# naimnv/cugraph-forked

Measured on AMD Instinct MI355X. Metric: PageRank edges/sec + BFS MTEPS on RMAT-24 at 1/2/4/8 MI355X, higher is better.
Workload: dtype f32

## Files before the change

cugraph-forked_amd/csrc/capi.hpp:

```cpp
#pragma once

#include "common.hpp"

#include <cugraph_c/algorithms.h>

#include <memory>
#include <string>
#include <cstring>
#include <vector>

namespace cgx {

struct mg_graph_t;
struct mg_context;

struct tuning_t {
  int pr_win_bits      = 0;
  bool pr_packed       = true;
  bool pr_whole        = true;
  bool pr_calib        = true;
  bool pr_deal_global  = false;
  bool pr_unit_w       = true;
  bool pr_fuse         = true;
  bool pr_enc          = true;
  bool pr_hub          = true;
  int64_t pr_band_cut  = -1;
  int pr_perm          = -1;
  int64_t pr_perm_cut  = -1;
  int pr_perm_span     = -1;
  int pr_share_div     = 0;
  bool pr_fast_build   = true;
  int mg_chunks        = 0;
  double bfs_alpha     = 40.0;
  double bfs_beta      = 64.0;
  double mg_bfs_alpha  = 40.0;
  double mg_bfs_beta   = 64.0;
  int mg_bfs_pipelined = 1;
  bool bfs_probe_vec   = true;
  bool bfs_head        = true;
  int bfs_res_grid     = 1024;
  int bfs_probe_grid   = 4096;
  int64_t bfs_td_cap   = 1024;
  bool louvain_hash    = true;
  bool louvain_big_hash = true;
  int louvain_big_cap  = 0;
  int64_t louvain_big_maxdeg = 0;
  bool louvain_wide_keys = false;
  double sssp_delta    = 0;
  int sssp_pull        = 0;
  int wcc_sample       = 2;
  int tc_path          = 0;
};

struct handle_t {
  int device         = 0;
  hipStream_t stream = nullptr;
  mg_context* mg     = nullptr;
  bool profiling     = false;
  tuning_t tune;
  size_t last_iterations     = 0;
  double last_hot_ms         = 0;
  size_t last_hot_launches   = 0;
  int64_t last_pr_stream     = 0;
  int64_t last_pr_permuted   = 0;
  size_t last_bfs_levels    = 0;
  size_t last_bfs_bottom_up  = 0;
  size_t last_louvain_levels = 0;
  double last_louvain_sweep_bytes = 0;
  int64_t last_louvain_local_edges = 0;
  int64_t last_louvain_ghosts      = 0;
  void* pinned = nullptr;
  std::vector<hipEvent_t> events;
  template <typename T>
  T* pinned_as()
  {
    static_assert(sizeof(T) <= kPinnedBytes, "pinned scratch too small");
    if (!pinned) HIP_CHECK(hipHostMalloc(&pinned, kPinnedBytes, hipHostMallocDefault));
    return static_cast<T*>(pinned);
  }
  void* polled = nullptr;
  template <typename T>
  T* polled_as()
  {
    static_assert(sizeof(T) <= kPinnedBytes, "polled scratch too small");
    if (!polled) {
      HIP_CHECK(hipHostMalloc(&polled, kPinnedBytes, hipHostMallocCoherent));
      std::memset(polled, 0, kPinnedBytes);
    }
    return static_cast<T*>(polled);
  }
  hipEvent_t event(size_t i)
  {
    while (events.size() <= i) {
      hipEvent_t e;
      HIP_CHECK(hipEventCreate(&e));
      events.push_back(e);
    }
    return events[i];
  }
  static constexpr size_t kPinnedBytes = 4096;
  ~handle_t()
  {
    if (pinned) (void)hipHostFree(pinned);
    if (polled) (void)hipHostFree(polled);
    for (auto e : events) (void)hipEventDestroy(e);
  }
};

struct array_view_t {
  void* data           = nullptr;
  size_t size          = 0;
  size_t num_bytes     = 0;
  data_type_id_t type  = INT32;
  template <typename T>
  T* as() const
  {
    return static_cast<T*>(data);
  }
};

struct device_array_t {
  buffer buf;
  size_t size         = 0;
  data_type_id_t type = INT32;
  device_array_t(size_t n, data_type_id_t t, hipStream_t s) : buf(n * dtype_size(t), s), size(n), type(t) {}
  array_view_t view() const { return array_view_t{buf.data(), size, size * dtype_size(type), type}; }
};

struct host_array_t {
  std::vector<std::byte> data;
  size_t size         = 0;
  data_type_id_t type = INT32;
};

struct err_t {
  std::string message;
};

struct pr_push_t {
  bool built = false;
  bool ok    = false;
  int win_bits = 12;
  buffer ent;
  buffer ew;
  bool packed = false;
  buffer ent16;
  buffer seg_base;
  buffer units;
  int64_t nunits = 0;
  buffer acc;
  int64_t nacc = 0;
  buffer items;
  buffer queue;
  std::vector<int64_t> qoff;
  int64_t nitems = 0;
  int64_t nwin   = 0;
  buffer tile_ctr;
  buffer win_multi;
  buffer win_items;
  buffer win_left;
  buffer empty_wins;
  int64_t nempty = 0, nwin_items = 0;
  buffer item_ticks;
  int calib = 0;
  bool bands = false;
  int64_t nwin_real = 0;
  buffer win_pub;
  buffer carry;
  buffer pos;
  int64_t perm_cut = 0;
  int64_t stream_len = 0;
  int last_iters = 0;
  double last_alpha = -1.0, last_eps = -1.0;
};

constexpr int64_t kIdxPad = 16;

struct adjacency_t {
  buffer offsets;
  buffer indices;
  buffer weights;
  bool idx_padded = false;
  bool degree_sorted = false;
  int64_t max_degree = -1;
  int unit_weights   = -1;
  bool sched_valid   = false;
  buffer order;
  std::vector<int64_t> bin_begin;
  buffer items;
  int64_t num_items = 0;
  buffer bfs_head;
  double wsum = -1;
  double sssp_delta = -1;
  int64_t sssp_eL = 0, sssp_eH = 0;
  buffer sssp_offL, sssp_offH, sssp_idxL, sssp_wL, sssp_idxH, sssp_wH, sssp_crowL, sssp_crowH;
  int64_t tc_edges = -1;
  buffer tc_ooff;
  buffer tc_oidx;
  pr_push_t pr;
};

struct graph_t {
  data_type_id_t vertex_type = INT32;
  data_type_id_t edge_type   = INT32;
  data_type_id_t weight_type = FLOAT32;
  bool store_transposed      = false;
  bool symmetric             = false;
  bool multigraph            = false;
  bool weighted              = false;
  bool renumbered            = false;
  bool multi_gpu             = false;
  int64_t num_vertices       = 0;
  int64_t num_edges          = 0;
  std::shared_ptr<adjacency_t> out;
  std::shared_ptr<adjacency_t> in;
  buffer number_map;
  bool ext_lookup_valid = false;
  buffer ext_sorted;
  buffer ext_internal;
  bool outw_valid = false;
  buffer outw;
  std::shared_ptr<mg_graph_t> mg;
};

struct centrality_result_t {
  std::unique_ptr<device_array_t> vertices;
  std::unique_ptr<device_array_t> values;
};

struct labeling_result_t {
  std::unique_ptr<device_array_t> vertices;
  std::unique_ptr<device_array_t> labels;
};

struct triangle_count_result_t {
  std::unique_ptr<device_array_t> vertices;
  std::unique_ptr<device_array_t> counts;
};

struct paths_result_t {
  std::unique_ptr<device_array_t> vertices;
  std::unique_ptr<device_array_t> distances;
  std::unique_ptr<device_array_t> predecessors;
};

struct extract_paths_result_t {
  size_t max_path_length = 0;
  std::unique_ptr<device_array_t> paths;
};

struct hits_result_t {
  std::unique_ptr<device_array_t> vertices;
  std::unique_ptr<device_array_t> hubs;
  std::unique_ptr<device_array_t> authorities;
  double hub_score_differences = 0;
  size_t number_of_iterations  = 0;
};

struct clustering_result_t {
  std::unique_ptr<device_array_t> vertices;
  std::unique_ptr<device_array_t> clusters;
  double modularity = 0;
  std::vector<std::unique_ptr<device_array_t>> levels;
};

inline handle_t* H(cugraph_resource_handle_t const* h) { return reinterpret_cast<handle_t*>(const_cast<cugraph_resource_handle_t*>(h)); }
inline graph_t* G(cugraph_graph_t* g) { return reinterpret_cast<graph_t*>(g); }
inline graph_t const* G(cugraph_graph_t const* g) { return reinterpret_cast<graph_t const*>(g); }
inline array_view_t const* AV(cugraph_type_erased_device_array_view_t const* v)
{
  return reinterpret_cast<array_view_t const*>(v);
}
inline array_view_t* AV(cugraph_type_erased_device_array_view_t* v) { return reinterpret_cast<array_view_t*>(v); }

inline cugraph_type_erased_device_array_view_t* new_view(device_array_t const* a)
{
  return reinterpret_cast<cugraph_type_erased_device_array_view_t*>(new array_view_t(a->view()));
}

template <typename F>
cugraph_error_code_t guarded(cugraph_error_t** error, F&& f)
{
  try {
    f();
    return CUGRAPH_SUCCESS;
  } catch (cgx::error const& e) {
    if (error) *error = reinterpret_cast<cugraph_error_t*>(new err_t{e.what()});
    return e.code;
  } catch (std::bad_alloc const& e) {
    if (error) *error = reinterpret_cast<cugraph_error_t*>(new err_t{std::string("allocation failed: ") + e.what()});
    return CUGRAPH_ALLOC_ERROR;
  } catch (std::exception const& e) {
    if (error) *error = reinterpret_cast<cugraph_error_t*>(new err_t{e.what()});
    return CUGRAPH_UNKNOWN_ERROR;
  }
}

void build_sg_graph(handle_t& h, graph_t& g, array_view_t const& src, array_view_t const& dst,
                    array_view_t const* weights, bool renumber);
adjacency_t& ensure_adjacency(handle_t& h, graph_t& g, bool transposed);
void ensure_schedule(handle_t& h, graph_t& g, adjacency_t& adj);
void renumber_ext_to_int(handle_t& h, graph_t& g, void* ids, size_t n, bool check);
void renumber_ext_to_int_unchecked(handle_t& h, graph_t& g, void* ids, size_t n);
void ensure_ext_lookup(handle_t& h, graph_t& g);
void unrenumber_int_to_ext(handle_t& h, graph_t& g, void* ids, size_t n);
std::unique_ptr<device_array_t> number_map_copy(handle_t& h, graph_t& g);
void const* out_weight_sums(handle_t& h, graph_t& g);

}
```

cugraph-forked_amd/csrc/capi_core.cpp:

```cpp
#include "capi.hpp"
#include "comm.hpp"

#include <cugraph_amd/ext.h>

#include <cstdlib>
#include <cstring>
#include <mutex>
#include <new>
#include <vector>

using namespace cgx;

namespace {

std::mutex g_stream_mutex;
std::vector<std::pair<int, hipStream_t>> g_free_streams;

void release_stream(int device, hipStream_t s)
{
  std::lock_guard<std::mutex> lk(g_stream_mutex);
  g_free_streams.emplace_back(device, s);
}

hipStream_t make_stream(int& device)
// ... 334 lines not shown
    CGX_EXPECTS(ps->type == INT32 || ps->type == INT64, CUGRAPH_UNSUPPORTED_TYPE_COMBINATION,
                "vertex type must be INT32 or INT64");
    auto g              = std::make_unique<graph_t>();
    g->vertex_type      = ps->type;
    g->edge_type        = ps->size < (size_t)INT32_MAX ? ps->type : INT64;
    g->weight_type      = pw ? pw->type : FLOAT32;
    g->weighted         = pw != nullptr;
    g->store_transposed = store_transposed == TRUE;
    g->symmetric        = properties ? properties->is_symmetric == TRUE : false;
    g->multigraph       = properties ? properties->is_multigraph == TRUE : false;
    build_sg_graph(*H(handle), *g, *ps, *pd, pw, renumber == TRUE);
    (void)check;
    *graph = reinterpret_cast<cugraph_graph_t*>(g.release());
  });
}

extern "C" void cugraph_sg_graph_free(cugraph_graph_t* graph)
{
  auto* g = G(graph);
  if (!g) return;
  (void)hipDeviceSynchronize();
  delete g;
}

extern "C" int64_t cugraph_amd_graph_get_number_of_vertices(const cugraph_graph_t* graph)
{
  return G(graph)->num_vertices;
}
extern "C" int64_t cugraph_amd_graph_get_number_of_edges(const cugraph_graph_t* graph) { return G(graph)->num_edges; }
extern "C" bool_t cugraph_amd_graph_is_symmetric(const cugraph_graph_t* graph)
{
  return G(graph)->symmetric ? TRUE : FALSE;
}

extern "C" cugraph_error_code_t cugraph_amd_device_array_views_copy(
  const cugraph_resource_handle_t* handle,
  size_t n,
  cugraph_type_erased_device_array_view_t* const* dst,
  const cugraph_type_erased_device_array_view_t* const* src,
  cugraph_error_t** error)
{
  *error = nullptr;
  return guarded(error, [&] {
    for (size_t i = 0; i < n; ++i) {
      auto* d       = AV(dst[i]);
      auto const* v = AV(src[i]);
      CGX_INPUT(d->type == v->type, "Invalid input argument: type mismatch");
      CGX_INPUT(d->size == v->size, "Invalid input argument: size mismatch");
    }
    for (size_t i = 0; i < n; ++i) {
      auto* d       = AV(dst[i]);
      auto const* v = AV(src[i]);
      if (v->num_bytes) HIP_CHECK(hipMemcpyAsync(d->data, v->data, v->num_bytes, hipMemcpyDefault, H(handle)->stream));
    }
    HIP_CHECK(hipStreamSynchronize(H(handle)->stream));
  });
}

extern "C" cugraph_error_code_t cugraph_amd_graph_get_adjacency(const cugraph_resource_handle_t* handle,
                                                               cugraph_graph_t* graph,
                                                               bool_t transposed,
                                                               cugraph_type_erased_device_array_t** offsets,
                                                               cugraph_type_erased_device_array_t** indices,
                                                               cugraph_type_erased_device_array_t** weights,
                                                               cugraph_error_t** error)
{
  *error = nullptr;
  return guarded(error, [&] {
    auto& h          = *H(handle);
    auto& g          = *G(graph);
    CGX_EXPECTS(!g.multi_gpu, CUGRAPH_NOT_IMPLEMENTED, "adjacency export is single-GPU only");
    adjacency_t& adj = ensure_adjacency(h, g, transposed == TRUE);
    size_t nv = (size_t)g.num_vertices, ne = (size_t)g.num_edges;
    auto o = new device_array_t(nv + 1, g.edge_type, h.stream);
    auto i = new device_array_t(ne, g.vertex_type, h.stream);
    HIP_CHECK(hipMemcpyAsync(o->buf.data(), adj.offsets.data(), (nv + 1) * dtype_size(g.edge_type),
                             hipMemcpyDeviceToDevice, h.stream));
    if (ne)
      HIP_CHECK(hipMemcpyAsync(i->buf.data(), adj.indices.data(), ne * dtype_size(g.vertex_type),
                               hipMemcpyDeviceToDevice, h.stream));
    *offsets = reinterpret_cast<cugraph_type_erased_device_array_t*>(o);
    *indices = reinterpret_cast<cugraph_type_erased_device_array_t*>(i);
    if (weights) {
      *weights = nullptr;
      if (g.weighted) {
        auto w = new device_array_t(ne, g.weight_type, h.stream);
        if (ne)
          HIP_CHECK(hipMemcpyAsync(w->buf.data(), adj.weights.data(), ne * dtype_size(g.weight_type),
                                   hipMemcpyDeviceToDevice, h.stream));
        *weights = reinterpret_cast<cugraph_type_erased_device_array_t*>(w);
      }
    }
    HIP_CHECK(hipStreamSynchronize(h.stream));
  });
}

extern "C" cugraph_error_code_t cugraph_amd_graph_get_out_weight_sums(const cugraph_resource_handle_t* handle,
                                                                     cugraph_graph_t* graph,
                                                                     cugraph_type_erased_device_array_t** sums,
                                                                     cugraph_error_t** error)
{
  *error = nullptr;
  *sums  = nullptr;
  return guarded(error, [&] {
    auto& h = *H(handle);
    auto& g = *G(graph);
    CGX_EXPECTS(!g.multi_gpu, CUGRAPH_NOT_IMPLEMENTED, "out-weight sums export is single-GPU only");
    size_t const nv = (size_t)g.num_vertices;
    void const* src = nv ? out_weight_sums(h, g) : nullptr;
    auto a          = new device_array_t(nv, g.weight_type, h.stream);
    if (nv)
      HIP_CHECK(hipMemcpyAsync(a->buf.data(), src, nv * dtype_size(g.weight_type), hipMemcpyDeviceToDevice, h.stream));
    HIP_CHECK(hipStreamSynchronize(h.stream));
    *sums = reinterpret_cast<cugraph_type_erased_device_array_t*>(a);
  });
}

extern "C" void cugraph_amd_set_profiling(cugraph_resource_handle_t* handle, bool_t enable)
{
  H(handle)->profiling = enable == TRUE;
}

extern "C" cugraph_error_code_t cugraph_amd_set_option(cugraph_resource_handle_t* handle, const char* name,
                                                       double value, cugraph_error_t** error)
{
  *error = nullptr;
  return guarded(error, [&] {
    CGX_INPUT(handle && name, "Invalid input argument: handle and name must not be NULL");
    tuning_t& t = H(handle)->tune;
    std::string const n(name);
    auto b   = [&](bool& f) { f = value != 0.0; };
    auto i32 = [&](int& f) { f = (int)value; };
    if (n == "pr_win_bits") {
      CGX_INPUT(value == 0 || value == 12 || value == 13 || value == 14 || value == 15,
                "Invalid input argument: pr_win_bits must be 0, 12, 13, 14 or 15");
      i32(t.pr_win_bits);
    } else if (n == "pr_packed") b(t.pr_packed);
    else if (n == "pr_whole") b(t.pr_whole);
    else if (n == "pr_calib") b(t.pr_calib);
    else if (n == "pr_deal_global") b(t.pr_deal_global);
    else if (n == "pr_unit_w") b(t.pr_unit_w);
    else if (n == "pr_fuse") b(t.pr_fuse);
    else if (n == "pr_enc") b(t.pr_enc);
    else if (n == "pr_hub") b(t.pr_hub);
    else if (n == "pr_band_cut") t.pr_band_cut = (int64_t)value;
    else if (n == "pr_perm") {
      CGX_INPUT(value == -1 || value == 0 || value == 1, "Invalid input argument: pr_perm must be -1, 0 or 1");
      i32(t.pr_perm);
    } else if (n == "pr_perm_cut") t.pr_perm_cut = (int64_t)value;
    else if (n == "pr_perm_span") {
      CGX_INPUT(value >= -1 && value <= 65536, "Invalid input argument: pr_perm_span must be in [-1, 65536]");
      i32(t.pr_perm_span);
    }
    else if (n == "pr_fast_build") b(t.pr_fast_build);
    else if (n == "pr_share_div") i32(t.pr_share_div);
    else if (n == "mg_chunks") i32(t.mg_chunks);
    else if (n == "sssp_pull") i32(t.sssp_pull);
    else if (n == "sssp_delta") {
      CGX_INPUT(value >= 0, "Invalid input argument: sssp_delta must be >= 0");
      t.sssp_delta = value;
    }
    else if (n == "wcc_sample") {
      CGX_INPUT(value >= 0 && value <= 64, "Invalid input argument: wcc_sample must be in [0, 64]");
      i32(t.wcc_sample);
    }
    else if (n == "tc_path") {
      CGX_INPUT(value == 0 || value == 1 || value == 2, "Invalid input argument: tc_path must be 0, 1 or 2");
      i32(t.tc_path);
    }
    else if (n == "bfs_alpha") t.bfs_alpha = value;
    else if (n == "bfs_beta") t.bfs_beta = value;
    else if (n == "mg_bfs_alpha") t.mg_bfs_alpha = value;
    else if (n == "mg_bfs_beta") t.mg_bfs_beta = value;
    else if (n == "mg_bfs_pipelined") i32(t.mg_bfs_pipelined);
    else if (n == "bfs_probe_vec") b(t.bfs_probe_vec);
    else if (n == "bfs_head") b(t.bfs_head);
    else if (n == "bfs_res_grid") i32(t.bfs_res_grid);
    else if (n == "bfs_probe_grid") i32(t.bfs_probe_grid);
    else if (n == "bfs_td_cap") t.bfs_td_cap = (int64_t)value;
    else if (n == "louvain_hash") b(t.louvain_hash);
    else if (n == "louvain_big_hash") b(t.louvain_big_hash);
    else if (n == "louvain_big_cap") i32(t.louvain_big_cap);
    else if (n == "louvain_big_maxdeg") t.louvain_big_maxdeg = (int64_t)value;
    else if (n == "louvain_wide_keys") b(t.louvain_wide_keys);
    else if (n == "defaults") t = tuning_t{};
    else fail(CUGRAPH_INVALID_INPUT, "Invalid input argument: unknown option " + n);
  });
}
extern "C" size_t cugraph_amd_last_iterations(const cugraph_resource_handle_t* handle)
{
  return H(handle)->last_iterations;
}
extern "C" double cugraph_amd_last_hot_kernel_ms(const cugraph_resource_handle_t* handle)
{
  return H(handle)->last_hot_ms;
}
extern "C" size_t cugraph_amd_last_hot_kernel_launches(const cugraph_resource_handle_t* handle)
{
  return H(handle)->last_hot_launches;
}
extern "C" void cugraph_amd_last_pagerank_schedule(const cugraph_resource_handle_t* handle, int64_t* stream_entries,
                                                   int64_t* permuted_vertices)
{
  *stream_entries    = H(handle)->last_pr_stream;
  *permuted_vertices = H(handle)->last_pr_permuted;
}
extern "C" size_t cugraph_amd_last_bfs_levels(const cugraph_resource_handle_t* handle)
{
  return H(handle)->last_bfs_levels;
}
extern "C" size_t cugraph_amd_last_bfs_bottom_up_steps(const cugraph_resource_handle_t* handle)
{
  return H(handle)->last_bfs_bottom_up;
}
extern "C" size_t cugraph_amd_last_louvain_levels(const cugraph_resource_handle_t* handle)
{
  return H(handle)->last_louvain_levels;
}
extern "C" double cugraph_amd_last_louvain_sweep_bytes(const cugraph_resource_handle_t* handle)
{
  return H(handle)->last_louvain_sweep_bytes;
}
extern "C" void cugraph_amd_last_louvain_partition(const cugraph_resource_handle_t* handle, int64_t* local_edges,
                                                   int64_t* ghosts)
{
  *local_edges = H(handle)->last_louvain_local_edges;
  *ghosts      = H(handle)->last_louvain_ghosts;
}
extern "C" size_t cugraph_amd_trim_device_cache(void) { return cgx::device_cache_trim(); }
extern "C" void cugraph_amd_allocator_stats(double* out) { cgx::device_alloc_stats(out); }
extern "C" const char* cugraph_amd_version(void) { return "cugraph-forked_amd libcugraph_c gfx950 " __DATE__; }
```

cugraph-forked_amd/csrc/pagerank.hip:

```cpp
#include "capi.hpp"
#include "comm.hpp"
#include "mg_graph.hpp"
#include "prims.hpp"
#include "schedule.hpp"

#include <rocprim/device/device_reduce_by_key.hpp>
#include <rocprim/iterator/counting_iterator.hpp>
#include <rocprim/iterator/transform_iterator.hpp>

#include <algorithm>
#include <cmath>
#include <cstdlib>

#if defined(__HIP_DEVICE_COMPILE__) && !defined(__GFX9__)
#error "s_waitcnt vmcnt(0) orders stores on gfx9-family (gfx950) targets only"
#endif

namespace cgx {

struct pr_state {
  double base;
  double pers_factor;
  double diff;
  double prev_diff;
// ... 236 lines not shown
      s1 += (double)x1 * (double)a.wgt[e + w];
    } else {
      s0 += (double)x0;
      s1 += (double)x1;
    }
  }
  if (e < end) {
    R x0 = a.x_in[a.idx[e]];
    if constexpr (WEIGHTED) s0 += (double)x0 * (double)a.wgt[e];
    else s0 += (double)x0;
  }
  return s0 + s1;
}

template <typename V, typename E, typename R, bool WEIGHTED>
__device__ __forceinline__ double row_partial_block(pr_args<V, E, R> const& a, E beg, E end, int tid)
{
  double s0 = 0, s1 = 0, s2 = 0, s3 = 0;
  E e = beg + tid;
  for (; e + 3 * 256 < end; e += 4 * 256) {
    V u0 = a.idx[e], u1 = a.idx[e + 256], u2 = a.idx[e + 512], u3 = a.idx[e + 768];
    R x0 = a.x_in[u0], x1 = a.x_in[u1], x2 = a.x_in[u2], x3 = a.x_in[u3];
    if constexpr (WEIGHTED) {
      s0 += (double)x0 * (double)a.wgt[e];
      s1 += (double)x1 * (double)a.wgt[e + 256];
      s2 += (double)x2 * (double)a.wgt[e + 512];
      s3 += (double)x3 * (double)a.wgt[e + 768];
    } else {
      s0 += (double)x0;
      s1 += (double)x1;
      s2 += (double)x2;
      s3 += (double)x3;
    }
  }
  for (; e < end; e += 256) {
    R x0 = a.x_in[a.idx[e]];
    if constexpr (WEIGHTED) s0 += (double)x0 * (double)a.wgt[e];
    else s0 += (double)x0;
  }
  return (s0 + s1) + (s2 + s3);
}

template <typename V, typename E, typename R, typename Acc = unsigned long long>
__device__ __forceinline__ void vertex_update_from(pr_args<V, E, R> const& a, V v, double s, R old, R ow, double base,
                                                   double pf, Acc& my_diff, Acc& my_dang)
{
  double n = base + a.alpha * s;
  if (a.pers) n += pf * (double)a.pers[v];
  R nr     = (R)n;
  a.pr[v]  = nr;
  acc_add(my_diff, fabs((double)nr - (double)old));
  R xv = R(0);
  if (ow == R(0)) acc_add(my_dang, (double)nr);
  else xv = (R)((double)nr / (double)ow);
  store_x<R>(a.x_out, x_index(a, (int64_t)v), xv, a.enc);
}

template <typename V, typename E, typename R, typename Acc = unsigned long long>
__device__ __forceinline__ void vertex_update(pr_args<V, E, R> const& a, V v, double s, double base, double pf,
                                              Acc& my_diff, Acc& my_dang)
{
  vertex_update_from<V, E, R, Acc>(a, v, s, a.pr[v], a.outw[v], base, pf, my_diff, my_dang);
}

template <typename V, typename E, typename R, bool WEIGHTED>
__global__ __launch_bounds__(256) void k_pr_iter(pr_args<V, E, R> a)
{
  __shared__ double sm[4];
  if (a.st->done) return;
  work_item const it = a.items[blockIdx.x];
  double const base  = a.st->base;
  double const pf    = a.st->pers_factor;
  double my_diff = 0, my_dang = 0;
  int const tid = threadIdx.x;
  if (it.width == 256) {
    for (int64_t p = it.begin; p < it.end; ++p) {
      V v      = a.order ? a.order[p] : (V)p;
      double s = row_partial_block<V, E, R, WEIGHTED>(a, a.off[v], a.off[v + 1], tid);
      s        = block_sum_256(s, sm);
      if (tid == 0) vertex_update<V, E, R, double>(a, v, s, base, pf, my_diff, my_dang);
    }
  } else {
    int const w      = it.width;
    int const lane   = tid & (w - 1);
    int const group  = tid / w;
    int const groups = 256 / w;
    for (int64_t p0 = it.begin; p0 < it.end; p0 += groups) {
      int64_t p  = p0 + group;
      bool valid = p < it.end;
      double s   = 0;
      V v        = 0;
      if (valid) {
        v = a.order ? a.order[p] : (V)p;
        s = row_partial<V, E, R, WEIGHTED>(a, a.off[v], a.off[v + 1], lane, w);
      }
      for (int o = w >> 1; o > 0; o >>= 1) s += __shfl_xor(s, o, 64);
      if (valid && lane == 0) vertex_update<V, E, R, double>(a, v, s, base, pf, my_diff, my_dang);
    }
  }
  finish_iteration<V, E, R>(a, my_diff, my_dang, true);
}

constexpr int kPushThreads = 1024;
constexpr int kPerThread   = 8;
constexpr int kPushUnit    = kPerThread * kPushThreads;
constexpr int kQueues      = 8;
constexpr int kTileUnits   = 8;
constexpr int kGroupItems  = 128;
constexpr int kCtrStride   = 32;
constexpr int kPushBlocks  = 512;
constexpr int kCommCUs     = 16;
constexpr int kHubBytes = 32768 - 512;
#ifndef CGX_APPLY_BATCH
#define CGX_APPLY_BATCH 4
#endif
template <typename R>
__host__ __device__ constexpr double fix_scale()
{
  return sizeof(R) == 8 ? 4611686018427387904.0  : 4503599627370496.0 ;
}
template <typename R>
__host__ __device__ constexpr double fix_scale_inv()
{
  return 1.0 / fix_scale<R>();
}

inline int push_win_bits(int64_t n_rows, tuning_t const& tu, bool wide = false)
{
  if (tu.pr_win_bits == 12 || tu.pr_win_bits == 13 || tu.pr_win_bits == 14) return tu.pr_win_bits;
  if (tu.pr_win_bits == 15) return wide ? 15 : 14;
  if (n_rows >= (int64_t(1) << 24)) return wide ? 15 : 14;
  return n_rows >= (int64_t(1) << 23) ? 14 : n_rows >= (int64_t(1) << 22) ? 13 : 12;
}

inline int64_t push_band_cut(int64_t n, tuning_t const& tu)
{
  if (tu.pr_band_cut >= 0) return tu.pr_band_cut;
  (void)n;
  return 0;
}

inline bool push_perm_on(int win_bits, tuning_t const& tu)
{
  if (tu.pr_perm >= 0) return tu.pr_perm != 0;
  return win_bits == 14;
}
inline int push_perm_span(int win_bits, tuning_t const& tu)
{
  (void)win_bits;
  return tu.pr_perm_span >= 0 ? tu.pr_perm_span : 1;
}
constexpr int64_t kPermCut = int64_t(1) << 20;

inline int push_blocks(int win_bits) { return win_bits >= 14 ? kPushBlocks / 2 : kPushBlocks; }

constexpr int64_t kShareDiv = 4;

struct push_unit {
  int64_t k0, k1;
  int64_t base;
  int64_t win;
};

template <typename V, typename E, typename R>
struct push_args {
  pr_args<V, E, R> a;
  uint32_t const* ent;
  R const* ew;
  uint16_t const* ent16;
  uint32_t const* seg_base;
  push_unit const* units;
  int64_t nunits;
  unsigned long long* acc;
  uint32_t* carry;
  int64_t const* items;
  int64_t const* queue;
  int64_t qoff[kQueues + 1];
  int64_t nitems;
  unsigned int* tile_ctr;
  uint8_t const* win_multi;
  int keep_acc;
  int win_bits;
  int64_t nwin;
  int fuse;
  int parity;
  uint32_t* win_left;
  uint32_t const* win_items;
  int64_t const* empty_wins;
  int64_t nempty;
  int64_t nwin_items;
  int bands;
  int64_t nwin_real;
  uint32_t* win_pub;
  int64_t nhub;
  unsigned long long* tl;
  int64_t tl_cap;
  int launch;
  uint32_t* item_ticks;
};

template <typename T>
__device__ __forceinline__ T nt_load(T const* p)
{
  return __builtin_nontemporal_load(p);
}

template <typename R>
__device__ __forceinline__ unsigned long long to_fixed(double v)
{
  return (unsigned long long)__double2ll_rn(v * fix_scale<R>());
}

__device__ __forceinline__ unsigned long long to_fixed_f32(float x)
{
  float const y     = x * 1048576.0f;
  uint32_t const hi = (uint32_t)y;
  float const fr    = y - (float)hi;
  uint32_t const lo = (uint32_t)__builtin_rintf(fr * 4294967296.0f);
  return ((unsigned long long)hi << 32) | lo;
}

template <typename R>
__device__ __forceinline__ unsigned long long fixed_of(R x)
{
  if constexpr (std::is_same<R, float>::value) return to_fixed_f32(x);
  else return to_fixed<R>((double)x);
}

constexpr int64_t kWholeItem = int64_t(1) << 40;
constexpr int64_t kWinMask   = kWholeItem - 1;

template <int WB, typename V, typename E, typename R, typename A>
__device__ __forceinline__ void flush_window(push_args<V, E, R> const& sa, A* acc, int64_t win_w)
{
  __syncthreads();
  unsigned long long* g = sa.acc + ((win_w & kWinMask) << WB);
  if (win_w & kWholeItem) {
    for (int i = threadIdx.x; i < (1 << WB); i += kPushThreads) {
      g[i]   = (unsigned long long)acc[i];
      acc[i] = 0;
    }
  } else {
    for (int i = threadIdx.x; i < (1 << WB); i += kPushThreads) {
      unsigned long long v = (unsigned long long)acc[i];
      if (v) {
        atomicAdd(g + i, v);
        acc[i] = 0;
      }
    }
  }
  __syncthreads();
}

__device__ __forceinline__ void wait_vmem() { asm volatile("s_waitcnt vmcnt(0)" ::: "memory"); }

template <int WB, typename V, typename E, typename R, typename A>
__device__ __forceinline__ void apply_window(push_args<V, E, R> const& sa, int64_t w, A* lds,
                                             unsigned long long& my_diff, unsigned long long& my_dang)
{
  auto const& a     = sa.a;
  double const base = a.st->base;
  double const pf   = a.st->pers_factor;
  int64_t const v0  = w << WB;
  int const n       = (int)min((int64_t)1 << WB, a.nv - v0);
  constexpr int kB = WB >= 14 ? 4 : 1;
  for (int i0 = threadIdx.x; i0 < n; i0 += kB * kPushThreads) {
    unsigned long long f[kB];
    R old[kB], ow[kB];
#pragma unroll
    for (int j = 0; j < kB; ++j) {
      int const i = i0 + j * kPushThreads;
      if (i < n) {
        if (lds) {
          f[j]   = (unsigned long long)lds[i];
          lds[i] = 0;
        } else {
          f[j] = __hip_atomic_exchange(sa.acc + v0 + i, 0ull, __ATOMIC_RELAXED, __HIP_MEMORY_SCOPE_AGENT);
        }
        if constexpr (WB == 15)
          f[j] += (unsigned long long)__hip_atomic_exchange(sa.carry + v0 + i, 0u, __ATOMIC_RELAXED,
                                                            __HIP_MEMORY_SCOPE_AGENT) << 32;
        old[j] = a.pr[v0 + i];
        ow[j]  = a.outw[v0 + i];
      }
    }
#pragma unroll
    for (int j = 0; j < kB; ++j) {
      int const i = i0 + j * kPushThreads;
      if (i < n)
        vertex_update_from<V, E, R>(a, (V)(v0 + i), (double)(long long)f[j] * fix_scale_inv<R>(), old[j], ow[j], base, pf,
                                    my_diff, my_dang);
    }
  }
}

template <int WB, typename V, typename E, typename R>
__device__ __forceinline__ void apply_window_banded(push_args<V, E, R> const& sa, int64_t rw, unsigned long long* lds,
                                                    int64_t own_vw, unsigned long long& my_diff,
                                                    unsigned long long& my_dang)
{
  auto const& a     = sa.a;
  double const base = a.st->base;
  double const pf   = a.st->pers_factor;
  int64_t const v0  = rw << WB;
  int const n       = (int)min((int64_t)1 << WB, a.nv - v0);
  int64_t const vw0 = rw, vw1 = rw + sa.nwin_real;
  bool const multi0 = sa.win_multi[vw0] != 0, multi1 = sa.win_multi[vw1] != 0;
  unsigned long long* const p0 = sa.acc + (vw0 << WB);
  unsigned long long* const p1 = sa.acc + (vw1 << WB);
  auto plane = [&](unsigned long long* p, bool multi, int i) -> unsigned long long {
    return multi ? __hip_atomic_exchange(p + i, 0ull, __ATOMIC_RELAXED, __HIP_MEMORY_SCOPE_AGENT)
                 : __hip_atomic_load(p + i, __ATOMIC_RELAXED, __HIP_MEMORY_SCOPE_AGENT);
  };
  constexpr int kB = 2;
  for (int i0 = threadIdx.x; i0 < n; i0 += kB * kPushThreads) {
    unsigned long long f[kB];
    R old[kB], ow[kB];
#pragma unroll
    for (int j = 0; j < kB; ++j) {
      int const i = i0 + j * kPushThreads;
      if (i < n) {
        unsigned long long x0, x1;
        if (lds && own_vw == vw0) {
// ... 147 lines not shown
    fused_finish<WB, V, E, R, true>(sa, acc, win_w);
    return;
  }
  if constexpr (FUSE) {
    if (sa.fuse) {
      fused_finish<WB, V, E, R>(sa, acc, win_w);
      return;
    }
  }
  flush_window<WB, V, E, R>(sa, acc, win_w);
}

template <int WB, typename V, typename E, typename R, bool WEIGHTED>
__device__ __forceinline__ void push_body(push_args<V, E, R> const& sa)
{
  constexpr int kWin = 1 << WB;
  __shared__ unsigned long long acc[kWin];
  __shared__ int64_t s_item;
  __shared__ unsigned long long s_t0;
  if (sa.a.st->done) return;
  int const tid = threadIdx.x;
  for (int i = tid; i < kWin; i += kPushThreads) acc[i] = 0ull;
  using cunit_t        = __attribute__((address_space(4))) push_unit const;
  cunit_t* const units = (cunit_t*)sa.units;
  R const* const x     = sa.a.x_in;
  int q                = (int)(blockIdx.x % kQueues);
  for (int tries = 0; tries < kQueues;) {
    if (tid == 0) {
      if (sa.item_ticks) s_t0 = __builtin_amdgcn_s_memrealtime();
      int64_t const i = (int64_t)atomicAdd(sa.tile_ctr + (sa.parity * kQueues + q) * kCtrStride, 1u);
      s_item          = i < sa.qoff[q + 1] - sa.qoff[q] ? sa.queue[sa.qoff[q] + i] : -1;
    }
    __syncthreads();
    int64_t const it = s_item;
    __syncthreads();
    if (it < 0) {
      q = (q + 1) % kQueues;
      ++tries;
      continue;
    }
    int64_t const ua = sa.items[it], ub = sa.items[it + 1];
    int64_t const win = units[ua].win;
    int64_t k0   = units[ua].k0;
    int n        = (int)(units[ua].k1 - k0);
    int64_t base = units[ua].base;
    uint32_t ent[kPerThread];
    R w[kPerThread];
#pragma unroll
    for (int j = 0; j < kPerThread; ++j) {
      ent[j] = nt_load(sa.ent + k0 + j * kPushThreads + tid);
      if constexpr (WEIGHTED) w[j] = nt_load(sa.ew + k0 + j * kPushThreads + tid);
    }
    for (int64_t un = ua; un < ub; ++un) {
      R const* const xb = x + base;
      R xv[kPerThread];
#pragma unroll
      for (int j = 0; j < kPerThread; ++j) {
        bool const ok = j * kPushThreads + tid < n;
        xv[j]         = xb[ok ? (ent[j] >> WB) : 0u];
        xv[j]         = ok ? xv[j] : R(0);
      }
      int64_t const nx  = un + 1 < ub ? un + 1 : un;
      int64_t const k0n = units[nx].k0;
      int const nn      = (int)(units[nx].k1 - k0n);
      int64_t const bsn = units[nx].base;
      uint32_t ent_n[kPerThread];
      R w_n[kPerThread];
#pragma unroll
      for (int j = 0; j < kPerThread; ++j) {
        ent_n[j] = nt_load(sa.ent + k0n + j * kPushThreads + tid);
        if constexpr (WEIGHTED) w_n[j] = nt_load(sa.ew + k0n + j * kPushThreads + tid);
      }
      __builtin_amdgcn_sched_barrier(0);
#pragma unroll
      for (int j = 0; j < kPerThread; ++j) {
        if constexpr (WEIGHTED) {
          atomicAdd(&acc[ent[j] & (kWin - 1)], to_fixed<R>((double)xv[j] * (double)w[j]));
        } else {
          atomicAdd(&acc[ent[j] & (kWin - 1)], fixed_of(xv[j]));
        }
      }
#pragma unroll
      for (int j = 0; j < kPerThread; ++j) {
        ent[j] = ent_n[j];
        if constexpr (WEIGHTED) w[j] = w_n[j];
      }
      n    = nn;
      base = bsn;
    }
    end_item<WB, V, E, R, (WB >= 14)>(sa, acc, win);
    if (sa.item_ticks && tid == 0) sa.item_ticks[s_item] = (uint32_t)(__builtin_amdgcn_s_memrealtime() - s_t0);
  }
}

template <int WB, typename V, typename E, typename R, bool WEIGHTED>
__global__ __launch_bounds__(kPushThreads, 8) void k_pr_push_q(push_args<V, E, R> sa)
{
  push_body<WB, V, E, R, WEIGHTED>(sa);
}

template <int WB, typename V, typename E, typename R, bool WEIGHTED>
__global__ __launch_bounds__(kPushThreads) void k_pr_push_q_wide(push_args<V, E, R> sa)
{
  push_body<WB, V, E, R, WEIGHTED>(sa);
}

constexpr int kSegEntries = 512;
typedef unsigned int u32x4_t __attribute__((ext_vector_type(4)));

__host__ __device__ __forceinline__ int64_t seg_store_index(int64_t p)
{
  int64_t const e = p & (kSegEntries - 1);
  return (p & ~(int64_t)(kSegEntries - 1)) | ((e & 63) << 3) | (e >> 6);
}
constexpr int kSegsPerUnit = kPushUnit / kSegEntries;

__device__ __forceinline__ uint32_t wave_incl_scan(uint32_t v)
{
  v += (uint32_t)__builtin_amdgcn_update_dpp(0, (int)v, 0x111, 0xf, 0xf, false);
  v += (uint32_t)__builtin_amdgcn_update_dpp(0, (int)v, 0x112, 0xf, 0xf, false);
  v += (uint32_t)__builtin_amdgcn_update_dpp(0, (int)v, 0x114, 0xf, 0xf, false);
  v += (uint32_t)__builtin_amdgcn_update_dpp(0, (int)v, 0x118, 0xf, 0xf, false);
  v += (uint32_t)__builtin_amdgcn_update_dpp(0, (int)v, 0x142, 0xa, 0xf, false);
  v += (uint32_t)__builtin_amdgcn_update_dpp(0, (int)v, 0x143, 0xc, 0xf, false);
  return v;
}

template <int N>
__device__ __forceinline__ void wave_incl_scan_rows(uint32_t (&v)[N])
{
#pragma unroll
  for (int j = 0; j < N; ++j) v[j] += (uint32_t)__builtin_amdgcn_update_dpp(0, (int)v[j], 0x111, 0xf, 0xf, false);
#pragma unroll
  for (int j = 0; j < N; ++j) v[j] += (uint32_t)__builtin_amdgcn_update_dpp(0, (int)v[j], 0x112, 0xf, 0xf, false);
#pragma unroll
  for (int j = 0; j < N; ++j) v[j] += (uint32_t)__builtin_amdgcn_update_dpp(0, (int)v[j], 0x114, 0xf, 0xf, false);
#pragma unroll
  for (int j = 0; j < N; ++j) v[j] += (uint32_t)__builtin_amdgcn_update_dpp(0, (int)v[j], 0x118, 0xf, 0xf, false);
#pragma unroll
  for (int j = 0; j < N; ++j) v[j] += (uint32_t)__builtin_amdgcn_update_dpp(0, (int)v[j], 0x142, 0xa, 0xf, false);
#pragma unroll
  for (int j = 0; j < N; ++j) v[j] += (uint32_t)__builtin_amdgcn_update_dpp(0, (int)v[j], 0x143, 0xc, 0xf, false);
}

template <int WB, typename V, typename E, typename R, bool ENC, bool HUB = false, bool FUSE = false, bool BANDS = false>
__device__ __forceinline__ void push_body16(push_args<V, E, R> const& sa)
{
  using xw_t = typename std::conditional<ENC, uint32_t, R>::type;
  constexpr int kWin        = 1 << WB;
  constexpr uint32_t kJump  = (1u << (16 - WB)) - 1;
  constexpr uint32_t kLow   = (1u << WB) - 1;
  constexpr int kRows       = kSegEntries / 64;
  static_assert(kRows == kPerThread, "a wave segment is one unit row per thread");
  constexpr bool kAcc32 = WB == 15;
  using acc_t           = typename std::conditional<kAcc32, uint32_t, unsigned long long>::type;
  __shared__ acc_t acc[kWin];
  constexpr int kHub = HUB ? kHubBytes / (int)sizeof(xw_t) : 1;
  __shared__ xw_t hub[kHub];
  __shared__ int64_t s_item;
  __shared__ unsigned long long s_t0;
  if (sa.a.st->done) return;
  int const tid  = threadIdx.x;
  int const lane = tid & 63;
  int const wave = __builtin_amdgcn_readfirstlane(tid >> 6);
  for (int i = tid; i < kWin; i += kPushThreads) acc[i] = 0;
  using cunit_t        = __attribute__((address_space(4))) push_unit const;
  cunit_t* const units = (cunit_t*)sa.units;
  xw_t const* const x  = reinterpret_cast<xw_t const*>(sa.a.x_in);
  uint32_t const nh    = HUB ? (uint32_t)min((int64_t)kHub, sa.nhub) : 0u;
  if constexpr (HUB)
    for (uint32_t i = tid; i < nh; i += kPushThreads) hub[i] = x[i];
  int q                = (int)(blockIdx.x % kQueues);
  for (int tries = 0; tries < kQueues;) {
    if (tid == 0) {
      if (sa.tl || sa.item_ticks) s_t0 = __builtin_amdgcn_s_memrealtime();
      int64_t const i = (int64_t)atomicAdd(sa.tile_ctr + (sa.parity * kQueues + q) * kCtrStride, 1u);
      s_item          = i < sa.qoff[q + 1] - sa.qoff[q] ? sa.queue[sa.qoff[q] + i] : -1;
    }
    __syncthreads();
    int64_t const it = s_item;
    __syncthreads();
    if (it < 0) {
      q = (q + 1) % kQueues;
      ++tries;
      continue;
    }
    int64_t const ua = sa.items[it], ub = sa.items[it + 1];
    int64_t const win = units[ua].win;
    auto seg_ptr = [&](int64_t u) {
      return reinterpret_cast<u32x4_t const*>(sa.ent16 + units[u].k0 + wave * kSegEntries) + lane;
    };
    auto seg_n = [&](int64_t u) { return (int)(units[u].k1 - units[u].k0) - wave * kSegEntries; };
    auto entry = [&](u32x4_t const& w, int j) { return (w[j >> 1] >> ((j & 1) * 16)) & 0xFFFFu; };
    auto gather = [&](u32x4_t const& w, uint32_t base, xw_t (&xv)[kRows]) {
      uint32_t sc[kRows];
#pragma unroll
      for (int j = 0; j < kRows; ++j) {
        uint32_t const e = entry(w, j);
        sc[j]            = (e >> WB) == kJump ? (e & kLow) : (e >> WB);
      }
      wave_incl_scan_rows<kRows>(sc);
      uint32_t run = base;
      if constexpr (HUB) {
        uint32_t src[kRows];
#pragma unroll
        for (int j = 0; j < kRows; ++j) {
          src[j] = run + sc[j];
          run += (uint32_t)__builtin_amdgcn_readlane((int)sc[j], 63);
        }
        if (run < nh) {
#pragma unroll
          for (int j = 0; j < kRows; ++j) xv[j] = hub[src[j]];
        } else {
#pragma unroll
          for (int j = 0; j < kRows; ++j) xv[j] = x[src[j]];
        }
        return;
      }
#pragma unroll
      for (int j = 0; j < kRows; ++j) {
        uint32_t const src = run + sc[j];
        run += (uint32_t)__builtin_amdgcn_readlane((int)sc[j], 63);
        xv[j] = x[src];
      }
    };
    auto sum = [&](u32x4_t const& w, xw_t const (&xv)[kRows]) {
      if constexpr (kAcc32) {
        uint32_t lo[kRows], old[kRows];
        uint32_t* const cw = sa.carry + ((win & kWinMask) << WB);
#pragma unroll
        for (int j = 0; j < kRows; ++j) {
          uint32_t const e = entry(w, j);
          unsigned long long fix;
          if constexpr (ENC) fix = dec_fixed(xv[j]);
          else fix = fixed_of(xv[j]);
          lo[j] = (e >> WB) != kJump ? (uint32_t)fix : 0u;
          if ((e >> WB) != kJump) {
            old[j] = atomicAdd(&acc[e & kLow], lo[j]);
            if (fix >> 32) atomicAdd(cw + (e & kLow), (uint32_t)(fix >> 32));
          }
        }
#pragma unroll
        for (int j = 0; j < kRows; ++j) {
          uint32_t const e = entry(w, j);
          if ((e >> WB) != kJump && old[j] > ~lo[j]) atomicAdd(cw + (e & kLow), 1u);
        }
      } else {
#pragma unroll
        for (int j = 0; j < kRows; ++j) {
          uint32_t const e = entry(w, j);
          xw_t const v     = xv[j];
          unsigned long long fix;
          if constexpr (ENC) fix = dec_fixed(v);
          else fix = fixed_of(v);
          if ((e >> WB) != kJump) atomicAdd(&acc[e & kLow], fix);
        }
      }
    };
    int64_t const u1 = ua + 1 < ub ? ua + 1 : ua;
    int nA      = seg_n(ua);
    int nB      = seg_n(u1);
    uint32_t bB = __builtin_amdgcn_readfirstlane(sa.seg_base[u1 * kSegsPerUnit + wave]);
    u32x4_t wA  = nt_load(seg_ptr(ua));
    u32x4_t wB  = nt_load(seg_ptr(u1));
    xw_t xA[kRows];
    if (nA > 0) gather(wA, __builtin_amdgcn_readfirstlane(sa.seg_base[ua * kSegsPerUnit + wave]), xA);
    for (int64_t un = ua; un < ub; ++un) {
      bool const actB = un + 1 < ub && nB > 0;
      xw_t xB[kRows];
      if (actB) gather(wB, bB, xB);
      int64_t const u2  = un + 2 < ub ? un + 2 : un;
      int const n2      = seg_n(u2);
      uint32_t const b2 = sa.seg_base[u2 * kSegsPerUnit + wave];
      u32x4_t const e2  = nt_load(seg_ptr(u2));
      __builtin_amdgcn_sched_barrier(0);
      if (nA > 0) sum(wA, xA);
      wA = wB;
#pragma unroll
      for (int j = 0; j < kRows; ++j) xA[j] = xB[j];
      nA = actB ? nB : 0;
      wB = e2;
      nB = n2;
      bB = __builtin_amdgcn_readfirstlane(b2);
    }
    end_item<WB, V, E, R, FUSE, BANDS>(sa, acc, win);
    if (sa.item_ticks && tid == 0) sa.item_ticks[s_item] = (uint32_t)(__builtin_amdgcn_s_memrealtime() - s_t0);
    if (sa.tl && tid == 0) {
      unsigned long long const t_end = __builtin_amdgcn_s_memrealtime();
      unsigned long long const k     = atomicAdd(sa.tl, 1ull);
      if ((int64_t)k < sa.tl_cap) {
        unsigned long long* r = sa.tl + 1 + 4 * k;
        r[0] = ((unsigned long long)sa.launch << 32) | blockIdx.x;
        int64_t const iu = s_item;
        r[1] = ((unsigned long long)(units[sa.items[iu + 1] - 1].k1 - units[sa.items[iu]].k0) << 32) | (unsigned long long)iu;
        r[2] = s_t0;
        r[3] = t_end;
      }
    }
  }
}

template <int WB, typename V, typename E, typename R, bool ENC>
__global__ __launch_bounds__(kPushThreads, 8) void k_pr_push16(push_args<V, E, R> sa)
{
  push_body16<WB, V, E, R, ENC>(sa);
}

template <typename V, typename E, typename R, bool ENC, bool BANDS = false>
__global__ __launch_bounds__(kPushThreads) void k_pr_push16_w14(push_args<V, E, R> sa)
{
  push_body16<14, V, E, R, ENC, true, true, BANDS>(sa);
}

template <typename V, typename E, typename R, bool ENC>
__global__ __launch_bounds__(kPushThreads) void k_pr_push16_w15(push_args<V, E, R> sa)
{
  push_body16<15, V, E, R, ENC, true, true, false>(sa);
}

template <typename V, typename E, typename R, bool WEIGHTED>
__global__ __launch_bounds__(kPushThreads) void k_pr_push_q_w14(push_args<V, E, R> sa)
{
  push_body<14, V, E, R, WEIGHTED>(sa);
}

template <typename V, typename E, typename R>
__global__ __launch_bounds__(256) void k_pr_apply(push_args<V, E, R> sa)
{
  auto const& a = sa.a;
  if (sa.tile_ctr && blockIdx.x == 0 && threadIdx.x < kQueues)
    sa.tile_ctr[(sa.parity * kQueues + threadIdx.x) * kCtrStride] = 0u;
  if (a.st->done) return;
  double const base = a.st->base;
  double const pf   = a.st->pers_factor;
  unsigned long long my_diff = 0, my_dang = 0;
  int64_t const stride = (int64_t)gridDim.x * blockDim.x;
  int64_t v            = blockIdx.x * (int64_t)blockDim.x + threadIdx.x;
  auto take_carry = [&](int64_t vv) -> unsigned long long {
    if (!sa.carry) return 0ull;
    uint32_t const c = sa.carry[vv];
    if (c) sa.carry[vv] = 0u;
    return (unsigned long long)c << 32;
  };
  if constexpr (std::is_same<R, float>::value) {
    typedef float f4_t __attribute__((ext_vector_type(4)));
    typedef unsigned u4_t __attribute__((ext_vector_type(4)));
    typedef unsigned long long u2_t __attribute__((ext_vector_type(2)));
    bool const aligned = ((reinterpret_cast<uintptr_t>(a.pr) | reinterpret_cast<uintptr_t>(a.outw) |
                           reinterpret_cast<uintptr_t>(a.x_out) | reinterpret_cast<uintptr_t>(sa.acc)) & 15) == 0 &&
                         !sa.carry;
    if (aligned) {
      int64_t const nq = a.nv / 4;
      for (int64_t q = v; q < nq; q += stride) {
        u2_t const f01 = reinterpret_cast<u2_t const*>(sa.acc)[2 * q];
        u2_t const f23 = reinterpret_cast<u2_t const*>(sa.acc)[2 * q + 1];
        f4_t const old = reinterpret_cast<f4_t const*>(a.pr)[q];
        f4_t const ow  = reinterpret_cast<f4_t const*>(a.outw)[q];
        unsigned long long const f[4] = {f01.x, f01.y, f23.x, f23.y};
        float const o[4] = {old.x, old.y, old.z, old.w}, w[4] = {ow.x, ow.y, ow.z, ow.w};
        float nr[4], xv[4];
#pragma unroll
        for (int j = 0; j < 4; ++j) {
          int64_t const vj = 4 * q + j;
          double n = base + a.alpha * ((double)(long long)f[j] * fix_scale_inv<R>());
          if (a.pers) n += pf * (double)a.pers[vj];
          nr[j] = (float)n;
          acc_add(my_diff, fabs((double)nr[j] - (double)o[j]));
          xv[j] = 0.0f;
          if (w[j] == 0.0f) acc_add(my_dang, (double)nr[j]);
          else xv[j] = (float)((double)nr[j] / (double)w[j]);
          if (!sa.keep_acc && f[j] && (!sa.win_multi || sa.win_multi[vj >> sa.win_bits])) sa.acc[vj] = 0ull;
        }
        reinterpret_cast<f4_t*>(a.pr)[q] = f4_t{nr[0], nr[1], nr[2], nr[3]};
        if (a.pos) {
          u4_t const p = reinterpret_cast<u4_t const*>(a.pos)[q];
          uint32_t const v4 = (uint32_t)(4 * q);
          if (p.x != v4 || p.y != v4 + 1 || p.z != v4 + 2 || p.w != v4 + 3) {
            store_x<R>(a.x_out, p.x, xv[0], a.enc);
            store_x<R>(a.x_out, p.y, xv[1], a.enc);
            store_x<R>(a.x_out, p.z, xv[2], a.enc);
            store_x<R>(a.x_out, p.w, xv[3], a.enc);
            continue;
          }
        }
        if (a.enc)
          reinterpret_cast<u4_t*>(a.x_out)[q] = u4_t{enc_fixed(xv[0]), enc_fixed(xv[1]), enc_fixed(xv[2]), enc_fixed(xv[3])};
        else
          reinterpret_cast<f4_t*>(a.x_out)[q] = f4_t{xv[0], xv[1], xv[2], xv[3]};
      }
      v = 4 * nq + blockIdx.x * (int64_t)blockDim.x + threadIdx.x;
    }
  }
  constexpr int kApplyBatch = CGX_APPLY_BATCH;
  for (; v + (kApplyBatch - 1) * stride < a.nv; v += kApplyBatch * stride) {
    unsigned long long f[kApplyBatch];
    R old[kApplyBatch], ow[kApplyBatch];
#pragma unroll
    for (int j = 0; j < kApplyBatch; ++j) {
      f[j]   = sa.acc[v + j * stride];
      old[j] = a.pr[v + j * stride];
      ow[j]  = a.outw[v + j * stride];
    }
#pragma unroll
    for (int j = 0; j < kApplyBatch; ++j) {
      int64_t const vj = v + j * stride;
      if (!sa.keep_acc && f[j] && (!sa.win_multi || sa.win_multi[vj >> sa.win_bits])) sa.acc[vj] = 0ull;
      f[j] += take_carry(vj);
      vertex_update_from<V, E, R>(a, (V)vj, (double)(long long)f[j] * fix_scale_inv<R>(), old[j], ow[j], base, pf, my_diff,
                                  my_dang);
    }
  }
  for (; v < a.nv; v += stride) {
    unsigned long long f = sa.acc[v];
    if (!sa.keep_acc && f && (!sa.win_multi || sa.win_multi[v >> sa.win_bits])) sa.acc[v] = 0ull;
    f += take_carry(v);
    vertex_update<V, E, R>(a, (V)v, (double)(long long)f * fix_scale_inv<R>(), base, pf, my_diff, my_dang);
  }
  finish_iteration<V, E, R>(a, my_diff, my_dang, true);
}

constexpr int kRowsTile = 4096;
template <typename E>
__device__ __forceinline__ int64_t row_of_edge(E const* off, int64_t lo, int64_t hi, int64_t e)
{
  while (lo < hi) {
    int64_t const mid = (lo + hi + 1) >> 1;
    if ((int64_t)off[mid] <= e) lo = mid;
    else hi = mid - 1;
  }
  return lo;
}

template <typename E>
__global__ __launch_bounds__(256) void k_edge_rows(E const* off, int64_t nv, int64_t ne, uint32_t* rows)
{
  __shared__ int64_t s_r[2];
  __shared__ E s_off[kRowsTile + 1];
  for (int64_t e0 = (int64_t)blockIdx.x * kRowsTile; e0 < ne; e0 += (int64_t)gridDim.x * kRowsTile) {
    int64_t const e1 = min(e0 + kRowsTile, ne);
    if (threadIdx.x == 0) {
      s_r[0] = row_of_edge(off, 0, nv - 1, e0);
      s_r[1] = row_of_edge(off, s_r[0], nv - 1, e1 - 1);
    }
    __syncthreads();
    int64_t const r0 = s_r[0], r1 = s_r[1];
    bool const staged = r1 - r0 < kRowsTile;
    if (staged)
// ... 146 lines not shown
  }
}

template <typename KC = key_w32>
__global__ void k_jump_counts(uint64_t const* keys, int64_t ne, int64_t const* ws, uint32_t dmax, uint32_t pmax,
                              uint32_t* mj, KC kc = {})
{
  for (int64_t k = blockIdx.x * (int64_t)blockDim.x + threadIdx.x; k < ne; k += (int64_t)gridDim.x * blockDim.x) {
    int64_t const w     = kc.win(keys[k]);
    uint32_t const prev = k == ws[w] ? 0u : kc.src(keys[k - 1]);
    uint32_t const D    = kc.src(keys[k]) - prev;
    mj[k]               = D > dmax ? (D + pmax - 1) / pmax : 0u;
  }
}

struct jump_count_p {
  uint64_t const* keys;
  int64_t const* ws;
  int64_t ne;
  key_p kc;
  uint32_t dmax, pmax;
  __device__ __forceinline__ uint32_t operator()(int64_t k) const
  {
    if (k >= ne) return 0u;
    uint64_t const key  = keys[k];
    int64_t const w     = kc.win(key);
    uint32_t const prev = k == ws[w] ? 0u : kc.src(keys[k - 1]);
    uint32_t const D    = kc.src(key) - prev;
    return D > dmax ? (D + pmax - 1) / pmax : 0u;
  }
};

__global__ void k_pack16(uint64_t const* keys, uint32_t const* vals, uint32_t const* rows, int64_t ne,
                         int64_t const* ws, uint32_t const* mj, unsigned long long const* cm,
                         unsigned long long const* pb, int wb, uint32_t pmax,
                         uint16_t* ent16)
{
  uint32_t const jump = (1u << (16 - wb)) - 1, low = (1u << wb) - 1;
  for (int64_t k = blockIdx.x * (int64_t)blockDim.x + threadIdx.x; k < ne; k += (int64_t)gridDim.x * blockDim.x) {
    int64_t const w     = (int64_t)(keys[k] >> 32);
    uint32_t const prev = k == ws[w] ? 0u : (uint32_t)keys[k - 1];
    uint32_t const D    = (uint32_t)keys[k] - prev;
    uint32_t const m    = mj[k];
    int64_t const pos   = k + (int64_t)cm[k] + (int64_t)pb[w];
    uint32_t const slot = rows[vals[k]] & low;
    if (m == 0) {
      ent16[seg_store_index(pos)] = (uint16_t)((D << wb) | slot);
    } else {
      for (uint32_t j = 0; j < m; ++j) {
        uint32_t const pay                  = j + 1 < m ? pmax : D - pmax * (m - 1);
        ent16[seg_store_index(pos - m + j)] = (uint16_t)((jump << wb) | pay);
      }
      ent16[seg_store_index(pos)] = (uint16_t)slot;
    }
  }
}

template <typename CM>
__global__ void k_pack16_p(uint64_t const* keys, int64_t ne, int64_t const* ws, CM const* cm,
                           unsigned long long const* pb, key_p kc, uint32_t pmax, uint16_t* ent16)
{
  int const wb        = kc.wb;
  uint32_t const jump = (1u << (16 - wb)) - 1;
  for (int64_t k = blockIdx.x * (int64_t)blockDim.x + threadIdx.x; k < ne; k += (int64_t)gridDim.x * blockDim.x) {
    uint64_t const key  = keys[k];
    int64_t const w     = kc.win(key);
    uint32_t const prev = k == ws[w] ? 0u : kc.src(keys[k - 1]);
    uint32_t const D    = kc.src(key) - prev;
    uint32_t const m    = (uint32_t)(cm[k] - cm[k - 1]);
    int64_t const pos   = k + (int64_t)cm[k] + (int64_t)pb[w];
    uint32_t const slot = kc.slot(key);
    if (m == 0) {
      ent16[seg_store_index(pos)] = (uint16_t)((D << wb) | slot);
    } else {
      for (uint32_t j = 0; j < m; ++j) {
        uint32_t const pay                  = j + 1 < m ? pmax : D - pmax * (m - 1);
        ent16[seg_store_index(pos - m + j)] = (uint16_t)((jump << wb) | pay);
      }
      ent16[seg_store_index(pos)] = (uint16_t)slot;
    }
  }
}

template <typename CM>
__device__ __forceinline__ int64_t packed_start(int64_t const* ws, CM const* cm, int64_t w, int64_t nwin, int64_t total)
{
  return w == nwin ? total : ws[w] + (ws[w] > 0 ? (int64_t)cm[ws[w] - 1] : 0);
}
template <typename CM>
__global__ void k_packed_pads(int64_t const* ws, CM const* cm, int64_t nwin, int64_t total, unsigned long long* pad)
{
  for (int64_t w = blockIdx.x * (int64_t)blockDim.x + threadIdx.x; w <= nwin; w += (int64_t)gridDim.x * blockDim.x) {
    int64_t const len = w == nwin ? 0 : packed_start(ws, cm, w + 1, nwin, total) - packed_start(ws, cm, w, nwin, total);
    pad[w]            = (unsigned long long)((kSegEntries - len % kSegEntries) % kSegEntries);
  }
}
template <typename CM>
__global__ void k_packed_win_starts(int64_t const* ws, CM const* cm, unsigned long long const* pb, int64_t nwin,
                                    int64_t total, int64_t* nws)
{
  for (int64_t w = blockIdx.x * (int64_t)blockDim.x + threadIdx.x; w <= nwin; w += (int64_t)gridDim.x * blockDim.x)
    nws[w] = packed_start(ws, cm, w, nwin, total) + (int64_t)pb[w];
}

__global__ void k_unit_counts(int64_t const* nws, int64_t nwin, uint32_t* cnt)
{
  for (int64_t w = blockIdx.x * (int64_t)blockDim.x + threadIdx.x; w <= nwin; w += (int64_t)gridDim.x * blockDim.x)
    cnt[w] = w == nwin ? 0u : (uint32_t)((nws[w + 1] - nws[w] + kPushUnit - 1) / kPushUnit);
}
__global__ void k_units_direct(int64_t const* nws, int64_t nwin, uint32_t const* upos, int64_t nunits,
                               push_unit* units)
{
  for (int64_t u = blockIdx.x * (int64_t)blockDim.x + threadIdx.x; u < nunits; u += (int64_t)gridDim.x * blockDim.x) {
    int64_t lo = 0, hi = nwin - 1;
    while (lo < hi) {
      int64_t const mid = (lo + hi + 1) >> 1;
      if ((int64_t)upos[mid] <= u) lo = mid;
      else hi = mid - 1;
    }
    units[u] = push_unit{nws[lo] + (u - (int64_t)upos[lo]) * kPushUnit, 0, 0, lo};
  }
}

__global__ void k_packed_unit_marks(int64_t const* nws, int64_t nwin, uint32_t* flag)
{
  for (int64_t w = blockIdx.x * (int64_t)blockDim.x + threadIdx.x; w < nwin; w += (int64_t)gridDim.x * blockDim.x)
    for (int64_t p = nws[w]; p < nws[w + 1]; p += kPushUnit) flag[p] = 1u;
}
__global__ void k_packed_unit_heads(uint32_t const* flag, uint32_t const* uid, int64_t total, int64_t const* nws,
                                    int64_t nwin, push_unit* units)
{
  for (int64_t p = blockIdx.x * (int64_t)blockDim.x + threadIdx.x; p < total; p += (int64_t)gridDim.x * blockDim.x) {
    if (!flag[p]) continue;
    int64_t lo = 0, hi = nwin - 1;
    while (lo < hi) {
      int64_t mid = (lo + hi + 1) >> 1;
      if (nws[mid] <= p) lo = mid;
      else hi = mid - 1;
    }
    units[uid[p]] = push_unit{p, 0, 0, lo};
  }
}

template <typename KC, typename CM>
__global__ void k_seg_bases(push_unit const* units, int64_t nunits, uint64_t const* keys, int64_t ne,
                            int64_t const* ws, uint32_t const* mj, CM const* cm, unsigned long long const* pb,
                            uint32_t dmax, uint32_t pmax, uint32_t* seg_base, KC kc)
{
  int64_t const n = nunits * kSegsPerUnit;
  for (int64_t i = blockIdx.x * (int64_t)blockDim.x + threadIdx.x; i < n; i += (int64_t)gridDim.x * blockDim.x) {
    push_unit const u = units[i / kSegsPerUnit];
    int64_t const p   = u.k0 + (i % kSegsPerUnit) * kSegEntries;
    uint32_t base     = 0;
    if (p < u.k1) {
      int64_t lo = 0, hi = ne - 1;
      while (lo < hi) {
        int64_t mid = (lo + hi) >> 1;
        if (mid + (int64_t)cm[mid] + (int64_t)pb[kc.win(keys[mid])] < p) lo = mid + 1;
        else hi = mid;
      }
      int64_t const k     = lo;
      uint32_t const m    = mj ? mj[k] : (uint32_t)(cm[k] - cm[k - 1]);
      int64_t const w     = kc.win(keys[k]);
      int64_t const j     = p - (k + (int64_t)cm[k] + (int64_t)pb[w] - m);
      uint32_t const prev = k == ws[w] ? 0u : kc.src(keys[k - 1]);
      uint32_t const src  = kc.src(keys[k]);
      uint32_t const D    = src - prev;
      base = j < (int64_t)m ? prev + pmax * (uint32_t)j : src - (m ? 0u : (D <= dmax ? D : 0u));
    }
    seg_base[i] = base;
  }
}

inline void mark_whole_items(hipStream_t s, pr_push_t& pp, push_unit* units, std::vector<push_unit>& hu,
                             std::vector<int64_t> const& item_u, int64_t nitems, tuning_t const& tu)
{
  int64_t const nunits = (int64_t)hu.size();
  bool const no_whole  = !tu.pr_whole;
  std::vector<uint8_t> multi((size_t)std::max<int64_t>(pp.nwin, 1), 0);
  for (int64_t i = 0; i < nitems; ++i) {
    int64_t const u = item_u[i], last = item_u[i + 1] - 1;
    int64_t const wu = hu[u].win & kWinMask;
    bool const whole = !no_whole && (u == 0 || (hu[u - 1].win & kWinMask) != wu) &&
                       (last + 1 >= nunits || (hu[last + 1].win & kWinMask) != wu);
    CGX_EXPECTS(!(hu[u].win & kWholeItem), CUGRAPH_UNKNOWN_ERROR, "mark_whole_items: unit already flagged");
    if (whole) hu[u].win |= kWholeItem;
    else multi[wu] = 1;
  }
  to_device(units, hu.data(), (size_t)nunits, s);
  {
    int64_t const nreal = pp.bands ? pp.nwin_real : pp.nwin;
    std::vector<uint32_t> cnt((size_t)std::max<int64_t>(nreal, 1), 0u);
    for (int64_t i = 0; i < nitems; ++i) {
      int64_t const wu = hu[item_u[i]].win & kWinMask;
      if (wu < pp.nwin) ++cnt[pp.bands ? wu % nreal : wu];
    }
    std::vector<int64_t> empty;
    pp.nwin_items = 0;
    for (int64_t w = 0; w < nreal; ++w) {
      if (cnt[w]) ++pp.nwin_items;
      else empty.push_back(w);
    }
    if (pp.bands) {
      pp.win_pub.set_stream(s);
      pp.win_pub.resize(cnt.size() * sizeof(uint32_t));
      HIP_CHECK(hipMemsetAsync(pp.win_pub.data(), 0, cnt.size() * sizeof(uint32_t), s));
    }
    pp.nempty = (int64_t)empty.size();
    pp.win_items.set_stream(s);
    pp.win_items.resize(cnt.size() * sizeof(uint32_t));
    to_device(pp.win_items.data<uint32_t>(), cnt.data(), cnt.size(), s);
    pp.win_left.set_stream(s);
    pp.win_left.resize(cnt.size() * sizeof(uint32_t));
    pp.empty_wins.set_stream(s);
    pp.empty_wins.resize(std::max<size_t>(empty.size(), 1) * sizeof(int64_t));
    if (!empty.empty()) to_device(pp.empty_wins.data<int64_t>(), empty.data(), empty.size(), s);
    HIP_CHECK(hipStreamSynchronize(s));
  }
  pp.win_multi.set_stream(s);
  pp.win_multi.resize(multi.size());
  to_device(pp.win_multi.data<uint8_t>(), multi.data(), multi.size(), s);
  HIP_CHECK(hipStreamSynchronize(s));
}

inline void upload_items(hipStream_t s, pr_push_t& pp, std::vector<int64_t> const& item_u,
                         std::vector<int64_t> const& queue, int64_t nitems)
{
  pp.items.set_stream(s);
  pp.items.resize(item_u.size() * sizeof(int64_t));
  to_device(pp.items.data<int64_t>(), item_u.data(), item_u.size(), s);
  pp.queue.set_stream(s);
  pp.queue.resize(std::max<size_t>(queue.size(), 1) * sizeof(int64_t));
  to_device(pp.queue.data<int64_t>(), queue.data(), queue.size(), s);
  pp.nitems = nitems;
}

inline void build_items(hipStream_t s, pr_push_t& pp, push_unit* units, int64_t nunits, bool xcd_queues,
                        tuning_t const& tu)
{
  int64_t const ne = nunits ? to_host(&units[nunits - 1].k1, 1, s)[0] : 0;
  auto hu = to_host(units, nunits, s);
  int64_t const div = tu.pr_share_div > 0 ? tu.pr_share_div : kShareDiv;
  int64_t const tg  = std::max<int64_t>(kPushUnit, ne / (push_blocks(pp.win_bits) * div));
  std::vector<int64_t> item_u, item_e;
  for (int64_t u0 = 0; u0 < nunits;) {
    int64_t u1 = u0;
    while (u1 < nunits && hu[u1].win == hu[u0].win) ++u1;
    int64_t const size = hu[u1 - 1].k1 - hu[u0].k0;
    int64_t const n    = std::max<int64_t>(1, (size + tg / 2) / tg);
    int64_t k          = 0;
    for (int64_t u = u0; u < u1; ++u) {
      int64_t const done = hu[u].k0 - hu[u0].k0;
      bool const head    = u == u0 || (xcd_queues ? (k < n && done * n >= k * size) : (u - u0) % kTileUnits == 0);
      if (head) {
        item_u.push_back(u);
        item_e.push_back(0);
        ++k;
      }
      item_e.back() += hu[u].k1 - hu[u].k0;
    }
    u0 = u1;
  }
  int64_t const nitems = (int64_t)item_u.size();
  item_u.push_back(nunits);
  std::vector<int64_t> queue;
  queue.reserve(nitems);
  if (xcd_queues) {
    int64_t const ngroups = (nitems + kGroupItems - 1) / kGroupItems;
    std::vector<int64_t> gsize(ngroups, 0), gorder(ngroups);
    for (int64_t i = 0; i < nitems; ++i) gsize[i / kGroupItems] += item_e[i];
    for (int64_t g = 0; g < ngroups; ++g) gorder[g] = g;
    std::stable_sort(gorder.begin(), gorder.end(), [&](int64_t a, int64_t b) { return gsize[a] > gsize[b]; });
    std::vector<int> gq(ngroups, 0);
    int64_t load[kQueues] = {};
    for (int64_t g : gorder) {
      int best = 0;
      for (int q = 1; q < kQueues; ++q)
        if (load[q] < load[best]) best = q;
      gq[g] = best;
      load[best] += gsize[g];
    }
    for (int q = 0; q < kQueues; ++q) {
      pp.qoff[q] = (int64_t)queue.size();
      for (int64_t i = 0; i < nitems; ++i)
        if (gq[i / kGroupItems] == q) queue.push_back(i);
    }
  } else {
    for (int64_t i = 0; i < nitems; ++i) queue.push_back(i);
    pp.qoff[0] = 0;
    for (int q = 1; q < kQueues; ++q) pp.qoff[q] = nitems;
  }
  pp.qoff[kQueues] = (int64_t)queue.size();
  mark_whole_items(s, pp, units, hu, item_u, nitems, tu);
  upload_items(s, pp, item_u, queue, nitems);
}

constexpr int kCalGroup = 16;

inline bool calibration_wanted(pr_push_t const& pp, tuning_t const& tu)
{
  return pp.calib == 0 && pp.nitems > 0 && tu.pr_calib;
}

inline void calibrate_queues(hipStream_t s, pr_push_t& pp, tuning_t const& tu)
{
  int64_t const n = pp.nitems;
  auto t          = to_host(pp.item_ticks.data<uint32_t>(), n, s);
  std::vector<int64_t> queue;
  queue.reserve(n);
  if (tu.pr_deal_global || pp.win_bits < 13) {
    for (int64_t i = 0; i < n; ++i) queue.push_back(i);
    std::stable_sort(queue.begin(), queue.end(), [&](int64_t a, int64_t b) { return t[a] > t[b]; });
    pp.qoff.assign(kQueues + 1, n);
    pp.qoff[0] = 0;
  } else {
    int64_t const G  = kCalGroup;
    int64_t const ng = (n + G - 1) / G;
    std::vector<uint64_t> gc(ng, 0);
    for (int64_t i = 0; i < n; ++i) gc[i / G] += t[i];
    std::vector<int64_t> go(ng);
    for (int64_t g = 0; g < ng; ++g) go[g] = g;
    std::stable_sort(go.begin(), go.end(), [&](int64_t a, int64_t b) { return gc[a] > gc[b]; });
    std::vector<std::vector<int64_t>> qg(kQueues);
    uint64_t load[kQueues] = {};
    for (int64_t g : go) {
      int best = 0;
      for (int q = 1; q < kQueues; ++q)
        if (load[q] < load[best]) best = q;
      qg[best].push_back(g);
      load[best] += gc[g];
    }
    if (pp.bands) {
      std::vector<int> gband(ng, 0);
      {
        auto hu = to_host(pp.units.data<push_unit>(), (size_t)pp.nunits, s);
        auto iu = to_host(pp.items.data<int64_t>(), (size_t)n, s);
        for (int64_t g = 0; g < ng; ++g) gband[g] = (hu[iu[g * G]].win & kWinMask) >= pp.nwin_real ? 1 : 0;
      }
      for (auto& l : qg) std::stable_sort(l.begin(), l.end(), [&](int64_t a, int64_t b) { return gband[a] < gband[b]; });
    }
    pp.qoff.assign(kQueues + 1, 0);
    for (int q = 0; q < kQueues; ++q) {
      pp.qoff[q] = (int64_t)queue.size();
      for (int64_t g : qg[q])
        for (int64_t i = g * G; i < std::min(n, (g + 1) * G); ++i) queue.push_back(i);
    }
    pp.qoff[kQueues] = n;
  }
  to_device(pp.queue.data<int64_t>(), queue.data(), queue.size(), s);
  HIP_CHECK(hipStreamSynchronize(s));
  pp.calib = 2;
}

template <typename C, typename R>
void build_push_from_coo(hipStream_t s, uint32_t const* rows, C const* cols, R const* w, int64_t ne, int64_t n_rows,
                         int64_t n_cols, pr_push_t& pp, tuning_t const& tu, bool col_sorted = false,
                         int64_t band_cut = 0, bool wide = false)
{
  pp.built = true;
  pp.ok    = (uint64_t)n_rows < (1ull << 32) && (uint64_t)n_cols < (1ull << 32) && (uint64_t)ne < (1ull << 32);
  if (!pp.ok) return;
  int const wb = push_win_bits(n_rows, tu, wide && !w && tu.pr_packed);
  int const sb = 32 - wb;
  if (wb != 14 || w || !tu.pr_packed || band_cut >= n_cols) band_cut = 0;
  pp.carry.release();
  pp.pos.release();
  pp.perm_cut   = 0;
  pp.stream_len = 0;
  int64_t const nwin_real = std::max<int64_t>(1, (n_rows + (int64_t(1) << wb) - 1) >> wb);
  int64_t const nwin      = band_cut > 0 ? 2 * nwin_real : nwin_real;
  pp.win_bits        = wb;
  pp.nwin            = nwin;
  pp.bands           = band_cut > 0;
  pp.nwin_real       = nwin_real;
  pp.nacc            = nwin << wb;
  pp.acc.set_stream(s);
  pp.acc.resize(pp.nacc * sizeof(unsigned long long));
  HIP_CHECK(hipMemsetAsync(pp.acc.data(), 0, pp.nacc * sizeof(unsigned long long), s));
  pp.tile_ctr.set_stream(s);
  pp.tile_ctr.resize(2 * kQueues * kCtrStride * sizeof(unsigned int));
  HIP_CHECK(hipMemsetAsync(pp.tile_ctr.data(), 0, 2 * kQueues * kCtrStride * sizeof(unsigned int), s));
  pp.nunits = 0;
  pp.nitems = 0;
  pp.qoff.assign(kQueues + 1, 0);
  if (ne == 0) return;
  dbuf<uint64_t> keys_out(ne, s);
  dbuf<uint32_t> vals_out(ne, s);
  {
    dbuf<uint64_t> keys(ne, s);
    dbuf<uint32_t> vals(ne, s);
    hipLaunchKernelGGL(k_push_keys<C>, dim3(grid_for(ne, kBlock, 16384)), dim3(kBlock), 0, s, cols, rows, ne, wb,
                       (uint32_t)band_cut, nwin_real, keys.data(), vals.data());
    CGX_LAUNCH_CHECK();
    radix_sort_pairs<uint64_t, uint32_t>(keys.data(), keys_out.data(), vals.data(), vals_out.data(), (size_t)ne,
                                         col_sorted ? 32 : 0,
                                         32 + bits_for((unsigned long long)std::max<int64_t>(nwin - 1, 1)), s);
  }
  dbuf<int64_t> ws(nwin + 1, s);
  hipLaunchKernelGGL(k_win_starts<key_w32>, dim3(grid_for(nwin + 1, kBlock, 4096)), dim3(kBlock), 0, s,
                     keys_out.data(), ne, nwin, ws.data(), key_w32{});
  CGX_LAUNCH_CHECK();
  pp.packed = false;
  if (!w && tu.pr_packed) {
    uint32_t const dmax = (1u << (16 - wb)) - 2;
    uint32_t const pmax = (1u << wb) - 1;
    dbuf<uint32_t> mj(ne + 1, s);
// ... 52 lines not shown
      pp.seg_base.resize(std::max<int64_t>(nunits * kSegsPerUnit, 1) * sizeof(uint32_t));
      hipLaunchKernelGGL((k_seg_bases<key_w32, unsigned long long>), dim3(grid_for(nunits * kSegsPerUnit, kBlock, 16384)), dim3(kBlock), 0, s, units,
                         nunits, keys_out.data(), ne, ws.data(), mj.data(), cm, pb.data(), dmax, pmax,
                         pp.seg_base.data<uint32_t>(), key_w32{});
      CGX_LAUNCH_CHECK();
      pp.ent.release();
      pp.ew.release();
      build_items(s, pp, units, nunits, wb >= 13, tu);
      pp.nunits = nunits;
      HIP_CHECK(hipStreamSynchronize(s));
      return;
    }
  }
  if (band_cut > 0 || wb == 15) {
    keys_out.free();
    vals_out.free();
    ws.free();
    build_push_from_coo<C, R>(s, rows, cols, w, ne, n_rows, n_cols, pp, tu, col_sorted, 0, false);
    return;
  }
  dbuf<uint32_t> flag(ne + 1, s), uid(ne + 1, s);
  hipLaunchKernelGGL(k_unit_flags, dim3(grid_for(ne, kBlock, 16384)), dim3(kBlock), 0, s, keys_out.data(), ne,
                     ws.data(), sb, flag.data());
  CGX_LAUNCH_CHECK();
  fill<uint32_t>(flag.data() + ne, 1, 0u, s);
  exclusive_scan<uint32_t, uint32_t>(flag.data(), uid.data(), ne + 1, s);
  int64_t const nunits = (int64_t)to_host(uid.data() + ne, 1, s)[0];
  pp.units.set_stream(s);
  pp.units.resize(std::max<int64_t>(nunits, 1) * sizeof(push_unit));
  push_unit* units = pp.units.data<push_unit>();
  hipLaunchKernelGGL(k_unit_heads, dim3(grid_for(ne, kBlock, 16384)), dim3(kBlock), 0, s, keys_out.data(),
                     flag.data(), uid.data(), ne, units);
  CGX_LAUNCH_CHECK();
  hipLaunchKernelGGL(k_unit_ends, dim3(grid_for(nunits, kBlock, 4096)), dim3(kBlock), 0, s, units, nunits, ne);
  CGX_LAUNCH_CHECK();
  pp.ent.set_stream(s);
  pp.ent.resize((ne + kPushUnit) * sizeof(uint32_t));
  HIP_CHECK(hipMemsetAsync(pp.ent.data<uint32_t>() + ne, 0, kPushUnit * sizeof(uint32_t), s));
  pp.ew.set_stream(s);
  if (w) {
    pp.ew.resize((ne + kPushUnit) * sizeof(R));
    HIP_CHECK(hipMemsetAsync(pp.ew.data<R>() + ne, 0, kPushUnit * sizeof(R), s));
  } else {
    pp.ew.release();
  }
  hipLaunchKernelGGL(k_push_pack<R>, dim3(grid_for(ne, kBlock, 16384)), dim3(kBlock), 0, s, keys_out.data(),
                     vals_out.data(), rows, w, flag.data(), uid.data(), units, ne, wb, pp.ent.data<uint32_t>(),
                     w ? pp.ew.data<R>() : nullptr);
  CGX_LAUNCH_CHECK();
  build_items(s, pp, units, nunits, wb >= 13, tu);
  pp.nunits = nunits;
  HIP_CHECK(hipStreamSynchronize(s));
}

template <typename R>
__global__ void k_count_non_unit(R const* w, size_t n, int* bad)
{
  int mine = 0;
  for (size_t i = blockIdx.x * (size_t)blockDim.x + threadIdx.x; i < n; i += (size_t)gridDim.x * blockDim.x)
    mine |= w[i] != R(1);
  if (__any(mine) && (threadIdx.x & 63) == 0) atomicOr(bad, 1);
}

template <typename R>
bool unit_weights(handle_t& h, graph_t& g, adjacency_t& adj)
{
  if (!g.weighted) return false;
  if (adj.unit_weights < 0) {
    hipStream_t s = h.stream;
    dbuf<int> bad(1, s);
    fill<int>(bad.data(), 1, 0, s);
    if (g.num_edges)
      hipLaunchKernelGGL(k_count_non_unit<R>, dim3(grid_for((size_t)g.num_edges, kBlock, 4096)), dim3(kBlock), 0, s,
                         adj.weights.data<R>(), (size_t)g.num_edges, bad.data());
    CGX_LAUNCH_CHECK();
    adj.unit_weights = (to_host_scalar(bad.data(), s) == 0 && h.tune.pr_unit_w) ? 1 : 0;
  }
  return adj.unit_weights == 1;
}

using window_sort_10 = rocprim::radix_sort_config<
    rocprim::default_config, rocprim::default_config,
    rocprim::radix_sort_onesweep_config<rocprim::kernel_config<1024, 8>, rocprim::kernel_config<1024, 8>, 10,
                                        rocprim::block_radix_rank_algorithm::match>>;
template <typename C>
void sort_window_keys(rocprim::double_buffer<uint64_t>& db, int64_t ne, int shv, int vbits, hipStream_t s)
{
  size_t tmp = 0;
  HIP_CHECK(rocprim::radix_sort_keys<C>(nullptr, tmp, db, (size_t)ne, shv, shv + vbits, s));
  buffer t(tmp, s);
  HIP_CHECK(rocprim::radix_sort_keys<C>(t.data(), tmp, db, (size_t)ne, shv, shv + vbits, s));
}

template <typename E>
__global__ void k_layout_keys(E const* off, uint32_t const* idx, int64_t cut, int64_t nv, int wb, int vb,
                              int64_t range_len, uint64_t* keys, uint32_t* ids)
{
  int64_t const n = nv - cut;
  for (int64_t i = blockIdx.x * (int64_t)blockDim.x + threadIdx.x; i < n; i += (int64_t)gridDim.x * blockDim.x) {
    int64_t const v = cut + i;
    int64_t const b = (int64_t)off[v], e = (int64_t)off[v + 1];
    uint64_t const w1 = e > b ? (uint64_t)(idx[e - 1] >> wb) : 0ull;
    uint64_t const w2 = e - b > 1 ? (uint64_t)(idx[e - 2] >> wb) : 0ull;
    uint64_t const r  = range_len ? (uint64_t)(i / range_len) : 0ull;
    keys[i]           = (r << (2 * vb)) | (w1 << vb) | w2;
    ids[i]            = (uint32_t)v;
  }
}

template <typename E>
__global__ void k_layout_finish(E const* off, uint32_t const* tail, int64_t cut, int64_t nv, uint32_t* pos,
                                uint32_t* inv, E* deg)
{
  for (int64_t p = blockIdx.x * (int64_t)blockDim.x + threadIdx.x; p <= nv; p += (int64_t)gridDim.x * blockDim.x) {
    if (p == nv) {
      deg[p] = E(0);
      continue;
    }
    int64_t const v = p < cut ? p : (int64_t)tail[p - cut];
    inv[p]          = (uint32_t)v;
    pos[v]          = (uint32_t)p;
    deg[p]          = off[v + 1] - off[v];
  }
}

template <typename E>
void build_x_layout(hipStream_t s, E const* off, uint32_t const* idx, int64_t nv, int wb, int64_t cut, int span,
                    pr_push_t& pp, dbuf<uint32_t>& inv, dbuf<E>& poff)
{
  int64_t const n    = nv - cut;
  int64_t const nwin = (nv + (int64_t(1) << wb) - 1) >> wb;
  int const vb       = std::max(1, bits_for((unsigned long long)std::max<int64_t>(nwin - 1, 1)));
  int64_t const range_len = span > 0 ? (int64_t)span << wb : 0;
  int const rb = range_len ? std::max(1, bits_for((unsigned long long)std::max<int64_t>((n - 1) / range_len, 1))) : 0;
  dbuf<uint64_t> k0(n, s), k1(n, s);
  dbuf<uint32_t> v0(n, s), v1(n, s);
  hipLaunchKernelGGL(k_layout_keys<E>, dim3(grid_for(n, kBlock, 4096)), dim3(kBlock), 0, s, off, idx, cut, nv, wb, vb,
                     range_len, k0.data(), v0.data());
  CGX_LAUNCH_CHECK();
  bool const in1 = radix_sort_pairs_db<uint64_t, uint32_t>(k0.data(), k1.data(), v0.data(), v1.data(), (size_t)n, 0,
                                                           rb + 2 * vb, s);
  pp.pos.set_stream(s);
  pp.pos.resize(nv * sizeof(uint32_t));
  inv.resize(nv, s);
  poff.resize(nv + 1, s);
  hipLaunchKernelGGL(k_layout_finish<E>, dim3(grid_for(nv + 1, kBlock, 4096)), dim3(kBlock), 0, s, off,
                     in1 ? v1.data() : v0.data(), cut, nv, pp.pos.data<uint32_t>(), inv.data(), poff.data());
  CGX_LAUNCH_CHECK();
  exclusive_scan<E, E>(poff.data(), poff.data(), (size_t)(nv + 1), s);
}

template <typename E, typename CM>
bool build_push_packed_sym_cm(hipStream_t s, E const* off, uint32_t const* idx, int64_t ne, int64_t nv, pr_push_t& pp,
                              tuning_t const& tu, int64_t band_cut, bool wide)
{
  int const wb = push_win_bits(nv, tu, wide);
  if (wb != 14 || band_cut >= nv) band_cut = 0;
  int64_t const nwin_real = std::max<int64_t>(1, (nv + (int64_t(1) << wb) - 1) >> wb);
  int64_t const nwin      = band_cut > 0 ? 2 * nwin_real : nwin_real;
  int const sbits = std::max(1, bits_for((unsigned long long)std::max<int64_t>(nv - 1, 1)));
  int const vbits = std::max(1, bits_for((unsigned long long)std::max<int64_t>(nwin - 1, 1)));
  int const shv   = wb + sbits;
  if (shv + vbits > 64 || (uint64_t)ne >= (1ull << 32) || (uint64_t)nv >= (1ull << 32)) return false;
  key_p const kc{shv, wb, (sbits >= 32 ? ~0ull : ((1ull << sbits) - 1ull))};
  uint32_t const dmax = (1u << (16 - wb)) - 2, pmax = (1u << wb) - 1;
  dbuf<uint32_t> inv;
  dbuf<E> poff;
  pp.pos.release();
  pp.perm_cut = 0;
  if (band_cut == 0 && ne && push_perm_on(wb, tu)) {
    int64_t const win = int64_t(1) << wb;
    int64_t cut       = std::min<int64_t>(std::max<int64_t>(tu.pr_perm_cut >= 0 ? tu.pr_perm_cut : kPermCut, 1), nv);
    cut               = (cut + win - 1) / win * win;
    if (cut < nv) {
      build_x_layout<E>(s, off, idx, nv, wb, cut, push_perm_span(wb, tu), pp, inv, poff);
      pp.perm_cut = cut;
    }
  }
  dbuf<uint64_t> kbuf(std::max<int64_t>(ne, 1), s);
  {
    dbuf<uint64_t> k2(std::max<int64_t>(ne, 1), s);
    if (ne) {
      hipLaunchKernelGGL(k_push_keys_p<E>, dim3((unsigned)std::min<int64_t>((ne + kRowsTile - 1) / kRowsTile, 65536)),
                         dim3(256), 0, s, off, idx, nv, ne, wb, shv, (uint32_t)band_cut, nwin_real, kbuf.data(),
                         pp.perm_cut ? poff.data() : (E const*)nullptr,
                         pp.perm_cut ? inv.data() : (uint32_t const*)nullptr);
      CGX_LAUNCH_CHECK();
      inv.free();
      poff.free();
      rocprim::double_buffer<uint64_t> db(kbuf.data(), k2.data());
      if (vbits <= 10) sort_window_keys<window_sort_10>(db, ne, shv, vbits, s);
      else sort_window_keys<rocprim::default_config>(db, ne, shv, vbits, s);
      if (db.current() != kbuf.data()) std::swap(kbuf, k2);
    }
  }
  uint64_t const* keys = kbuf.data();
  dbuf<int64_t> ws(nwin + 1, s);
  hipLaunchKernelGGL(k_win_starts<key_p>, dim3(grid_for(nwin + 1, kBlock, 4096)), dim3(kBlock), 0, s, keys, ne, nwin,
                     ws.data(), kc);
  CGX_LAUNCH_CHECK();
  dbuf<CM> ex(ne + 1, s);
  {
    auto jumps = rocprim::make_transform_iterator(rocprim::make_counting_iterator<int64_t>(0),
                                                  jump_count_p{keys, ws.data(), ne, kc, dmax, pmax});
    size_t tmp = 0;
    HIP_CHECK(rocprim::exclusive_scan(nullptr, tmp, jumps, ex.data(), CM(0), (size_t)(ne + 1), rocprim::plus<CM>(), s));
    buffer t(tmp, s);
    HIP_CHECK(rocprim::exclusive_scan(t.data(), tmp, jumps, ex.data(), CM(0), (size_t)(ne + 1), rocprim::plus<CM>(), s));
  }
  int64_t const total0 = ne + (int64_t)to_host(ex.data() + ne, 1, s)[0];
  CM const* cm         = ex.data() + 1;
  dbuf<unsigned long long> pad(nwin + 1, s), pb(nwin + 1, s);
  hipLaunchKernelGGL(k_packed_pads<CM>, dim3(grid_for(nwin + 1, kBlock, 4096)), dim3(kBlock), 0, s, ws.data(), cm, nwin,
                     total0, pad.data());
  CGX_LAUNCH_CHECK();
  exclusive_scan<unsigned long long, unsigned long long>(pad.data(), pb.data(), nwin + 1, s);
  int64_t const total = total0 + (int64_t)to_host(pb.data() + nwin, 1, s)[0];
  if (!(total <= ne + ne / 2 && (uint64_t)total < (1ull << 32))) {
    pp.pos.release();
    pp.perm_cut = 0;
    return false;
  }
  pp.built      = true;
  pp.ok         = true;
  pp.stream_len = total;
  pp.win_bits   = wb;
  pp.nwin      = nwin;
  pp.bands     = band_cut > 0;
  pp.nwin_real = nwin_real;
  pp.nacc      = nwin << wb;
  pp.acc.set_stream(s);
  pp.acc.resize(pp.nacc * sizeof(unsigned long long));
  HIP_CHECK(hipMemsetAsync(pp.acc.data(), 0, pp.nacc * sizeof(unsigned long long), s));
  pp.tile_ctr.set_stream(s);
  pp.tile_ctr.resize(2 * kQueues * kCtrStride * sizeof(unsigned int));
  HIP_CHECK(hipMemsetAsync(pp.tile_ctr.data(), 0, 2 * kQueues * kCtrStride * sizeof(unsigned int), s));
  pp.carry.release();
  if (wb == 15) {
    pp.carry.set_stream(s);
    pp.carry.resize(pp.nacc * sizeof(uint32_t));
    HIP_CHECK(hipMemsetAsync(pp.carry.data(), 0, pp.nacc * sizeof(uint32_t), s));
  }
  pp.qoff.assign(kQueues + 1, 0);
  pp.nitems = 0;
  pp.packed = true;
  uint16_t const pad_code = (uint16_t)(((1u << (16 - wb)) - 1) << wb);
  pp.ent16.set_stream(s);
  pp.ent16.resize((total + kPushUnit) * sizeof(uint16_t));
  fill<uint16_t>(pp.ent16.data<uint16_t>(), (size_t)(total + kPushUnit), pad_code, s);
  if (ne)
    hipLaunchKernelGGL(k_pack16_p<CM>, dim3(grid_for(ne, kBlock, 16384)), dim3(kBlock), 0, s, keys, ne, ws.data(),
                       cm, pb.data(), kc, pmax, pp.ent16.data<uint16_t>());
  CGX_LAUNCH_CHECK();
  dbuf<int64_t> nws(nwin + 1, s);
  hipLaunchKernelGGL(k_packed_win_starts<CM>, dim3(grid_for(nwin + 1, kBlock, 4096)), dim3(kBlock), 0, s, ws.data(),
                     cm, pb.data(), nwin, total0, nws.data());
  CGX_LAUNCH_CHECK();
  dbuf<uint32_t> ucnt(nwin + 1, s), upos(nwin + 1, s);
  hipLaunchKernelGGL(k_unit_counts, dim3(grid_for(nwin + 1, kBlock, 4096)), dim3(kBlock), 0, s, nws.data(), nwin,
                     ucnt.data());
  CGX_LAUNCH_CHECK();
  exclusive_scan<uint32_t, uint32_t>(ucnt.data(), upos.data(), nwin + 1, s);
  int64_t const nunits = (int64_t)to_host(upos.data() + nwin, 1, s)[0];
  pp.units.set_stream(s);
  pp.units.resize(std::max<int64_t>(nunits, 1) * sizeof(push_unit));
  push_unit* units = pp.units.data<push_unit>();
  if (nunits)
    hipLaunchKernelGGL(k_units_direct, dim3(grid_for(nunits, kBlock, 4096)), dim3(kBlock), 0, s, nws.data(), nwin,
                       upos.data(), nunits, units);
  CGX_LAUNCH_CHECK();
  hipLaunchKernelGGL(k_unit_ends, dim3(grid_for(nunits, kBlock, 4096)), dim3(kBlock), 0, s, units, nunits, total);
  CGX_LAUNCH_CHECK();
  pp.seg_base.set_stream(s);
  pp.seg_base.resize(std::max<int64_t>(nunits * kSegsPerUnit, 1) * sizeof(uint32_t));
  if (nunits)
    hipLaunchKernelGGL((k_seg_bases<key_p, CM>), dim3(grid_for(nunits * kSegsPerUnit, kBlock, 16384)), dim3(kBlock), 0,
                       s, units, nunits, keys, ne, ws.data(), (uint32_t const*)nullptr, cm, pb.data(), dmax, pmax,
                       pp.seg_base.data<uint32_t>(), kc);
  CGX_LAUNCH_CHECK();
  pp.ent.release();
  pp.ew.release();
  build_items(s, pp, units, nunits, wb >= 13, tu);
  pp.nunits = nunits;
  HIP_CHECK(hipStreamSynchronize(s));
  return true;
}

template <typename E>
bool build_push_packed_sym(hipStream_t s, E const* off, uint32_t const* idx, int64_t ne, int64_t nv, pr_push_t& pp,
                           tuning_t const& tu, int64_t band_cut, bool wide)
{
  if (ne < (int64_t(1) << 31)) return build_push_packed_sym_cm<E, uint32_t>(s, off, idx, ne, nv, pp, tu, band_cut, wide);
  return build_push_packed_sym_cm<E, unsigned long long>(s, off, idx, ne, nv, pp, tu, band_cut, wide);
}

template <typename V, typename E, typename R>
void build_pr_push_schedule(handle_t& h, graph_t& g, adjacency_t& adj, bool use_weights)
{
  hipStream_t s = h.stream;
  int64_t nv    = g.num_vertices;
  int64_t ne    = g.num_edges;
  if ((uint64_t)ne >= (1ull << 32) || (uint64_t)nv >= (1ull << 32)) {
    adj.pr.built = true;
    adj.pr.ok    = false;
    return;
  }
  if constexpr (sizeof(V) == 4) {
    if (g.symmetric && !use_weights && h.tune.pr_packed && h.tune.pr_fast_build &&
        build_push_packed_sym<E>(s, adj.offsets.data<E>(), reinterpret_cast<uint32_t const*>(adj.indices.data<V>()), ne,
                                 nv, adj.pr, h.tune, push_band_cut(nv, h.tune), sizeof(R) == 4))
      return;
  }
  dbuf<uint32_t> rows(std::max<int64_t>(ne, 1), s);
  if (ne)
    hipLaunchKernelGGL(k_edge_rows<E>, dim3((unsigned)std::min<int64_t>((ne + kRowsTile - 1) / kRowsTile, 65536)),
                       dim3(256), 0, s, adj.offsets.data<E>(), nv, ne, rows.data());
  CGX_LAUNCH_CHECK();
  if constexpr (sizeof(V) == 4) {
    if (g.symmetric) {
      build_push_from_coo<uint32_t, R>(s, reinterpret_cast<uint32_t const*>(adj.indices.data<V>()), rows.data(),
                                       use_weights ? adj.weights.data<R>() : nullptr, ne, nv, nv, adj.pr, h.tune,
                                       true, push_band_cut(nv, h.tune), sizeof(R) == 4);
      return;
    }
  }
  build_push_from_coo<V, R>(s, rows.data(), adj.indices.data<V>(), use_weights ? adj.weights.data<R>() : nullptr, ne,
                            nv, nv, adj.pr, h.tune, false, push_band_cut(nv, h.tune), sizeof(R) == 4);
}

template <typename V, typename R>
__global__ void k_scatter_values(R* dst, V const* ids, R const* vals, size_t n, double scale)
{
  for (size_t i = blockIdx.x * (size_t)blockDim.x + threadIdx.x; i < n; i += (size_t)gridDim.x * blockDim.x)
    dst[ids[i]] = (R)((double)vals[i] * scale);
}

template <typename R>
__global__ void k_count_negative(R const* p, size_t n, int* bad)
{
  for (size_t i = blockIdx.x * (size_t)blockDim.x + threadIdx.x; i < n; i += (size_t)gridDim.x * blockDim.x)
    if (p[i] < R(0)) atomicAdd(bad, 1);
}

template <typename R>
int count_negative(R const* p, size_t n, hipStream_t s)
{
  if (!n) return 0;
  dbuf<int> bad(1, s);
  fill<int>(bad.data(), 1, 0, s);
  hipLaunchKernelGGL(k_count_negative<R>, dim3(grid_for(n, kBlock, 4096)), dim3(kBlock), 0, s, p, n, bad.data());
  CGX_LAUNCH_CHECK();
  return to_host_scalar(bad.data(), s);
}

template <typename V, typename R>
dbuf<V> internal_ids(handle_t& h, graph_t& g, array_view_t const* ext)
{
  dbuf<V> ids(ext->size, h.stream);
  if (ext->size)
    HIP_CHECK(hipMemcpyAsync(ids.data(), ext->data, ext->size * sizeof(V), hipMemcpyDefault, h.stream));
  renumber_ext_to_int(h, g, ids.data(), ext->size, true);
  return ids;
}

template <typename V, typename E, typename R>
void set_queue_args(push_args<V, E, R>& sa, pr_push_t& pp, hipStream_t s)
{
  sa.ent      = pp.ent.data<uint32_t>();
  sa.ew       = pp.ew.empty() ? nullptr : pp.ew.data<R>();
  sa.ent16    = pp.ent16.data<uint16_t>();
  sa.seg_base = pp.seg_base.data<uint32_t>();
  sa.units    = pp.units.data<push_unit>();
  sa.nunits   = pp.nunits;
  sa.acc      = pp.acc.data<unsigned long long>();
  sa.carry    = pp.win_bits == 15 ? pp.carry.data<uint32_t>() : nullptr;
  sa.items    = pp.items.data<int64_t>();
  sa.queue    = pp.queue.data<int64_t>();
  sa.nitems   = pp.nitems;
  for (int q = 0; q <= kQueues; ++q) sa.qoff[q] = q < (int)pp.qoff.size() ? pp.qoff[q] : 0;
  sa.tile_ctr = pp.tile_ctr.data<unsigned int>();
  sa.nwin     = pp.nwin;
  HIP_CHECK(hipMemsetAsync(sa.tile_ctr, 0, 2 * kQueues * kCtrStride * sizeof(unsigned int), s));
  sa.fuse      = 0;
  sa.parity    = 0;
  sa.bands     = pp.bands ? 1 : 0;
  sa.nwin_real = pp.nwin_real;
  sa.win_pub   = pp.bands ? pp.win_pub.data<uint32_t>() : nullptr;
  if (!pp.win_items.empty()) {
    sa.win_items  = pp.win_items.data<uint32_t>();
    sa.win_left   = pp.win_left.data<uint32_t>();
    sa.empty_wins = pp.empty_wins.data<int64_t>();
    sa.nempty     = pp.nempty;
    sa.nwin_items = pp.nwin_items;
    int64_t const nreal = pp.bands ? pp.nwin_real : pp.nwin;
    HIP_CHECK(hipMemcpyAsync(sa.win_left, sa.win_items, nreal * sizeof(uint32_t), hipMemcpyDeviceToDevice, s));
    if (pp.bands) HIP_CHECK(hipMemsetAsync(sa.win_pub, 0, nreal * sizeof(uint32_t), s));
  }

}

inline bool fuse_apply(pr_push_t const& pp, tuning_t const& tu)
{
  if (pp.bands) return pp.nitems > 0;
  return pp.win_bits >= 14 && pp.nitems > 0 && pp.nwin_items > 0 && pp.nempty <= 64 && !pp.win_items.empty() &&
         tu.pr_fuse;
}

template <typename V, typename E, typename R>
auto push_kernel(pr_push_t const& pp, bool weighted, bool enc = false)
{
  if (pp.win_bits == 15) return enc ? k_pr_push16_w15<V, E, R, true> : k_pr_push16_w15<V, E, R, false>;
  if (pp.win_bits == 14) {
    if (pp.packed && pp.bands) return enc ? k_pr_push16_w14<V, E, R, true, true> : k_pr_push16_w14<V, E, R, false, true>;
    if (pp.packed) return enc ? k_pr_push16_w14<V, E, R, true> : k_pr_push16_w14<V, E, R, false>;
    return weighted ? k_pr_push_q_w14<V, E, R, true> : k_pr_push_q_w14<V, E, R, false>;
  }
  if (pp.packed) {
    if (enc) return pp.win_bits == 13 ? k_pr_push16<13, V, E, R, true> : k_pr_push16<12, V, E, R, true>;
    return pp.win_bits == 13 ? k_pr_push16<13, V, E, R, false> : k_pr_push16<12, V, E, R, false>;
  }
  constexpr bool wide = sizeof(R) == 8;
  if (pp.win_bits == 13)
    return weighted ? (wide ? k_pr_push_q_wide<13, V, E, R, true> : k_pr_push_q<13, V, E, R, true>)
                    : k_pr_push_q<13, V, E, R, false>;
  return weighted ? (wide ? k_pr_push_q_wide<12, V, E, R, true> : k_pr_push_q<12, V, E, R, true>)
                  : k_pr_push_q<12, V, E, R, false>;
}

template <typename V, typename E, typename R>
void pagerank_impl(handle_t& h, graph_t& g, array_view_t const* pow_v, array_view_t const* pow_s,
                   array_view_t const* guess_v, array_view_t const* guess_s, array_view_t const* pers_v,
                   array_view_t const* pers_s, double alpha, double eps, size_t max_iter, bool expensive,
                   centrality_result_t& res)
{
  hipStream_t s = h.stream;
  CGX_INPUT(alpha >= 0.0 && alpha <= 1.0, "Invalid input argument: alpha should be in [0.0, 1.0].");
  CGX_INPUT(eps >= 0.0, "Invalid input argument: epsilon should be non-negative.");
  CGX_INPUT((pers_v == nullptr) == (pers_s == nullptr) && (!pers_v || pers_v->size == pers_s->size),
            "Invalid input argument: personalization vertices and values must be given together.");
  CGX_INPUT((guess_v == nullptr) == (guess_s == nullptr), "Invalid input argument: initial guess vertices and values must be given together.");
  CGX_INPUT((pow_v == nullptr) == (pow_s == nullptr), "Invalid input argument: precomputed out weight vertices and sums must be given together.");
  int64_t nv = g.num_vertices;
  res.vertices = number_map_copy(h, g);
  res.values   = std::make_unique<device_array_t>((size_t)nv, dtype_of<R>(), s);
  h.last_iterations = 0;
  h.last_hot_ms     = 0;
  h.last_hot_launches = 0;
  if (nv == 0) return;

  adjacency_t& adj = ensure_adjacency(h, g, true);
  if (expensive && g.weighted) {
    CGX_INPUT(count_negative<R>(adj.weights.data<R>(), (size_t)g.num_edges, s) == 0,
              "Invalid input argument: input graph should have non-negative edge weights.");
  }

  dbuf<R> outw_own;
  R const* outw = nullptr;
  if (pow_v) {
    outw_own.resize(nv, s);
    fill<R>(outw_own.data(), nv, R(0), s);
    auto ids = internal_ids<V, R>(h, g, pow_v);
    if (pow_v->size)
      hipLaunchKernelGGL((k_scatter_values<V, R>), dim3(grid_for(pow_v->size, kBlock, 4096)), dim3(kBlock), 0, s,
                         outw_own.data(), ids.data(), pow_s->as<R>(), pow_v->size, 1.0);
    CGX_LAUNCH_CHECK();
    if (expensive)
      CGX_INPUT(count_negative<R>(outw_own.data(), nv, s) == 0,
                "Invalid input argument: outgoing edge weight sum values should be non-negative.");
    outw = outw_own.data();
  } else {
    outw = static_cast<R const*>(out_weight_sums(h, g));
  }

  R* pr = res.values->buf.data<R>();
  if (guess_v) {
    fill<R>(pr, nv, R(0), s);
    auto ids = internal_ids<V, R>(h, g, guess_v);
    auto hv  = to_host(guess_s->as<R>(), guess_s->size, s);
    double sum = 0;
    for (auto x : hv) sum += (double)x;
    if (expensive) {
      for (auto x : hv) CGX_INPUT(x >= R(0), "Invalid input argument: initial guess values should be non-negative.");
    }
    CGX_INPUT(sum > 0.0, "Invalid input argument: sum of the PageRank initial guess values should be positive.");
    if (guess_v->size)
      hipLaunchKernelGGL((k_scatter_values<V, R>), dim3(grid_for(guess_v->size, kBlock, 4096)), dim3(kBlock), 0, s,
                         pr, ids.data(), guess_s->as<R>(), guess_v->size, 1.0 / sum);
    CGX_LAUNCH_CHECK();
  } else {
    fill<R>(pr, nv, (R)(R(1.0) / (R)nv), s);
  }

  dbuf<R> pers;
  if (pers_v && pers_v->size > 0) {
    auto hv    = to_host(pers_s->as<R>(), pers_s->size, s);
    double sum = 0;
    for (auto x : hv) {
      if (expensive) CGX_INPUT(x >= R(0), "Invalid input argument: peresonalization values should be non-negative.");
      sum += (double)x;
    }
    CGX_INPUT(sum > 0.0, "Invalid input argument: sum of personalization valuese should be positive.");
    pers.resize(nv, s);
    fill<R>(pers.data(), nv, R(0), s);
    auto ids = internal_ids<V, R>(h, g, pers_v);
    hipLaunchKernelGGL((k_scatter_values<V, R>), dim3(grid_for(pers_v->size, kBlock, 4096)), dim3(kBlock), 0, s,
                       pers.data(), ids.data(), pers_s->as<R>(), pers_v->size, 1.0 / sum);
    CGX_LAUNCH_CHECK();
  }

  bool push = pow_v == nullptr && max_iter > 0;
  bool const push_w = g.weighted && !(push && unit_weights<R>(h, g, adj));
  if (push && !adj.pr.built) build_pr_push_schedule<V, E, R>(h, g, adj, push_w);
  push = push && adj.pr.ok;
  if (!push) ensure_schedule(h, g, adj);

  int const nblk_iter = push ? 0 : (int)adj.num_items;
  int const nblk_init = (int)grid_for(nv, kBlock, 1024);
  dbuf<double> partials(2 * std::max<int64_t>({nblk_iter, nblk_init, 2048, (nv + 4095) / 4096}), s);
  dbuf<pr_state> st(1, s);
  HIP_CHECK(hipMemsetAsync(st.data(), 0, sizeof(pr_state), s));
  dbuf<R> xa(nv, s), xb(nv, s);

  pr_args<V, E, R> a{};
  a.off      = adj.offsets.data<E>();
  a.idx      = adj.indices.data<V>();
  a.wgt      = g.weighted ? adj.weights.data<R>() : nullptr;
  a.order    = push || adj.degree_sorted ? nullptr : adj.order.data<V>();
  a.items    = push ? nullptr : adj.items.data<work_item>();
  a.pr       = pr;
  a.outw     = outw;
  a.pers     = pers.data();
  a.alpha    = alpha;
  a.eps      = eps;
  a.max_iter = (int)std::min<size_t>(max_iter, (size_t)INT32_MAX);
  a.nv       = nv;
  a.nv_global = nv;
  a.partials = partials.data();
  a.st       = st.data();
  a.x_in     = nullptr;
  a.x_out    = xa.data();

  a.enc  = push && adj.pr.packed && std::is_same<R, float>::value && h.tune.pr_enc;
  a.fp64 = push ? 0 : 1;
  a.pos  = push && adj.pr.perm_cut ? adj.pr.pos.data<uint32_t>() : nullptr;
  h.last_pr_stream   = push ? adj.pr.stream_len : 0;
  h.last_pr_permuted = push && adj.pr.perm_cut ? nv - adj.pr.perm_cut : 0;
  hipLaunchKernelGGL((k_pr_init<V, E, R>), dim3(nblk_init), dim3(kBlock), 0, s, a);
  CGX_LAUNCH_CHECK();

  if (max_iter == 0) fail(CUGRAPH_UNKNOWN_ERROR, "PageRank failed to converge.");

  push_args<V, E, R> sa{};
  int nblk_push = 0, nblk_apply = 0;
  bool const fuse = push && fuse_apply(adj.pr, h.tune);
  auto pkernel    = push_kernel<V, E, R>(adj.pr, push_w, a.enc != 0);
  if (push) {
    set_queue_args(sa, adj.pr, s);
    sa.win_multi = adj.pr.win_multi.data<uint8_t>();
    sa.win_bits  = adj.pr.win_bits;
    nblk_push  = sa.nitems ? push_blocks(sa.win_bits) : 0;
    nblk_apply = (int)grid_for(nv, kBlock, 512);
    sa.fuse    = fuse ? 1 : 0;
    sa.nhub    = h.tune.pr_hub ? nv : 0;
  }
  bool calibrating = push && calibration_wanted(adj.pr, h.tune);
  if (calibrating) {
    adj.pr.item_ticks.set_stream(s);
    adj.pr.item_ticks.resize(adj.pr.nitems * sizeof(uint32_t));
    HIP_CHECK(hipMemsetAsync(adj.pr.item_ticks.data(), 0, adj.pr.nitems * sizeof(uint32_t), s));
    adj.pr.calib = 1;
  } else if (push && adj.pr.calib == 0) {
    adj.pr.calib = 2;
  }
  char const* tl_path = push ? std::getenv("CGX_PR_TIMELINE") : nullptr;
  dbuf<unsigned long long> tl;
  if (tl_path) {
    sa.tl_cap = 1 << 20;
    tl.resize(1 + 4 * sa.tl_cap, s);
    HIP_CHECK(hipMemsetAsync(tl.data(), 0, sizeof(unsigned long long), s));
    sa.tl = tl.data();
  }
  std::vector<hipEvent_t> ev;
  pr_state hst{};
  R* bufs[2]    = {xa.data(), xb.data()};
  size_t launched = 0;
  bool const plain = push && !guess_v && !pers.data() && !calibrating;
  int const hint   = plain && adj.pr.last_alpha == alpha && adj.pr.last_eps == eps ? adj.pr.last_iters : 0;
  auto kernel  = g.weighted ? k_pr_iter<V, E, R, true> : k_pr_iter<V, E, R, false>;
  pr_state* hpin = h.pinned_as<pr_state>();
  while (true) {
    if (h.profiling) {
      ev.push_back(h.event(ev.size()));
      ev.push_back(h.event(ev.size()));
      HIP_CHECK(hipEventRecord(ev[ev.size() - 2], s));
    }
    int const chunk = launched == 0 && hint > 0 ? std::min(std::min(hint, 64), std::max(1, a.max_iter))
                                                : next_chunk(hst, eps, a.max_iter);
    for (int i = 0; i < chunk; ++i) {
      a.x_in  = bufs[launched & 1];
      a.x_out = bufs[(launched + 1) & 1];
      if (push) {
        sa.a          = a;
        sa.parity     = (int)(launched & 1);
        sa.launch     = (int)launched;
        sa.item_ticks = calibrating && launched == 0 ? adj.pr.item_ticks.data<uint32_t>() : nullptr;
        if (nblk_push) hipLaunchKernelGGL(pkernel, dim3(nblk_push), dim3(kPushThreads), 0, s, sa);
        if (!sa.fuse) hipLaunchKernelGGL((k_pr_apply<V, E, R>), dim3(nblk_apply), dim3(kBlock), 0, s, sa);
      } else {
        hipLaunchKernelGGL(kernel, dim3(nblk_iter), dim3(kBlock), 0, s, a);
      }
      CGX_LAUNCH_CHECK();
      ++launched;
    }
    if (h.profiling) HIP_CHECK(hipEventRecord(ev.back(), s));
    HIP_CHECK(hipMemcpyAsync(hpin, st.data(), sizeof(pr_state), hipMemcpyDeviceToHost, s));
    HIP_CHECK(hipStreamSynchronize(s));
    hst = *hpin;
    if (calibrating) {
      calibrate_queues(s, adj.pr, h.tune);
      for (int q = 0; q <= kQueues; ++q) sa.qoff[q] = adj.pr.qoff[q];
      calibrating = false;
    }
    if (hst.done) break;
  }
  h.last_iterations = (size_t)hst.iter;
  if (push && !guess_v && !pers.data()) {
    adj.pr.last_iters = hst.iter;
    adj.pr.last_alpha = alpha;
    adj.pr.last_eps   = eps;
  }
  if (tl_path) {
    unsigned long long n = 0;
    HIP_CHECK(hipMemcpyAsync(&n, tl.data(), sizeof(n), hipMemcpyDeviceToHost, s));
    HIP_CHECK(hipStreamSynchronize(s));
    n = std::min<unsigned long long>(n, (unsigned long long)sa.tl_cap);
    std::vector<unsigned long long> rec(4 * n);
    if (n) HIP_CHECK(hipMemcpyAsync(rec.data(), tl.data() + 1, rec.size() * sizeof(unsigned long long), hipMemcpyDeviceToHost, s));
    HIP_CHECK(hipStreamSynchronize(s));
    if (FILE* f = std::fopen(tl_path, "w")) {
      std::fprintf(f, "launch,block,item,entries,window,start,end\n");
      auto hu = to_host(adj.pr.units.data<push_unit>(), adj.pr.nunits, s);
      auto hi = to_host(adj.pr.items.data<int64_t>(), adj.pr.nitems + 1, s);
      for (unsigned long long i = 0; i < n; ++i) {
        unsigned long long const it = rec[4 * i + 1] & 0xffffffffull;
        std::fprintf(f, "%llu,%llu,%llu,%llu,%lld,%llu,%llu\n", rec[4 * i] >> 32, rec[4 * i] & 0xffffffffull, it,
                     rec[4 * i + 1] >> 32, (long long)(hu[hi[it]].win & kWinMask), rec[4 * i + 2], rec[4 * i + 3]);
      }
      std::fclose(f);
    }
  }
  if (h.profiling) {
    double tot = 0;
    for (size_t i = 0; i + 1 < ev.size(); i += 2) {
      float ms = 0;
      HIP_CHECK(hipEventElapsedTime(&ms, ev[i], ev[i + 1]));
      tot += ms;
    }
    h.last_hot_ms       = tot;
    h.last_hot_launches = std::max<size_t>((size_t)hst.iter, 1);
  }
  if (hst.done == 2) fail(CUGRAPH_UNKNOWN_ERROR, "PageRank failed to converge.");
}

struct mg_chunk {
  pr_push_t pp;
  dbuf<int64_t> multi_wins;
  int64_t nmulti = 0;
};

struct mg_pr_block {
  int64_t nmax_row = 0, nmax_col = 0;
  int K = 1;
  int64_t cs = 0;
  std::vector<mg_chunk> ch;
  buffer outw;
  hipStream_t comm_stream = nullptr;
  std::vector<hipEvent_t> ev;
  ~mg_pr_block()
  {
    for (auto e : ev) (void)hipEventDestroy(e);
    if (comm_stream) (void)hipStreamDestroy(comm_stream);
  }
};

__global__ void k_sorted_starts(uint32_t const* sorted, int64_t n, int K, int64_t* st)
{
  for (int k = threadIdx.x; k <= K; k += blockDim.x) {
    int64_t lo = 0, hi = n;
    while (lo < hi) {
      int64_t const mid = (lo + hi) >> 1;
      if ((int)sorted[mid] < k) lo = mid + 1;
      else hi = mid;
    }
    st[k] = lo;
  }
}

__global__ void k_mg_row_chunks(uint32_t* rows, int64_t ne, int64_t nmax_col, int64_t cs, uint32_t* chunk)
{
  for (int64_t e = blockIdx.x * (int64_t)blockDim.x + threadIdx.x; e < ne; e += (int64_t)gridDim.x * blockDim.x) {
    int64_t const q = rows[e] / nmax_col, l = rows[e] % nmax_col, k = l / cs;
    chunk[e] = (uint32_t)k;
    rows[e]  = (uint32_t)(q * cs + (l - k * cs));
  }
}

__global__ void k_clear_windows(unsigned long long* acc, int64_t const* wins, int64_t n, int wb)
{
  int64_t const per = int64_t(1) << wb;
  for (int64_t i = blockIdx.x * (int64_t)blockDim.x + threadIdx.x; i < n * per; i += (int64_t)gridDim.x * blockDim.x)
    acc[(wins[i >> wb] << wb) + (i & (per - 1))] = 0ull;
}

template <typename V>
__global__ void k_mg_block_coo(V const* src, V const* dst, int64_t ne, int64_t const* voff, int P, int C,
                               int64_t nmax_row, int64_t nmax_col, uint32_t* rows, uint32_t* cols)
{
  for (int64_t e = blockIdx.x * (int64_t)blockDim.x + threadIdx.x; e < ne; e += (int64_t)gridDim.x * blockDim.x) {
    int ou  = mg_owner_of_global((int64_t)src[e], voff, P);
    int ov  = mg_owner_of_global((int64_t)dst[e], voff, P);
    cols[e] = (uint32_t)((ou % C) * nmax_row + ((int64_t)src[e] - voff[ou]));
    rows[e] = (uint32_t)((ov / C) * nmax_col + ((int64_t)dst[e] - voff[ov]));
  }
}

template <typename R>
__global__ void k_weight_or_one(R const* w, int64_t n, double* out)
{
  for (int64_t i = blockIdx.x * (int64_t)blockDim.x + threadIdx.x; i < n; i += (int64_t)gridDim.x * blockDim.x)
    out[i] = w ? (double)w[i] : 1.0;
}

__global__ void k_scatter_sums(uint32_t const* keys, double const* vals, int64_t n, double* out)
{
  for (int64_t i = blockIdx.x * (int64_t)blockDim.x + threadIdx.x; i < n; i += (int64_t)gridDim.x * blockDim.x)
    out[keys[i]] = vals[i];
}

template <typename R>
__global__ void k_to_weight(double const* in, int64_t n, R* out)
{
  for (int64_t i = blockIdx.x * (int64_t)blockDim.x + threadIdx.x; i < n; i += (int64_t)gridDim.x * blockDim.x)
    out[i] = (R)in[i];
}

template <typename V, typename E, typename R>
__global__ void k_mg_finish_guarded(pr_args<V, E, R> a, bool count_iter)
{
  if (threadIdx.x == 0 && blockIdx.x == 0 && !a.st->done)
    update_state<V, E, R>(a, (double)a.mg_sums[0] * kSumScaleInv, (double)a.mg_sums[1] * kSumScaleInv, count_iter);
}

template <typename V, typename E, typename R>
mg_pr_block& mg_block(handle_t& h, graph_t& g)
{
  mg_graph_t& mg = *g.mg;
  if (mg.pr_block) return *static_cast<mg_pr_block*>(mg.pr_block.get());
  hipStream_t s = h.stream;
  mg_context& ctx = *h.mg;
  auto blk      = std::make_shared<mg_pr_block>();
  int const P = mg.P, C = mg.C, R_ = mg.R, r = mg.p / C, c = mg.p % C;
  for (int q = 0; q < C; ++q) blk->nmax_row = std::max(blk->nmax_row, mg.voff[r * C + q + 1] - mg.voff[r * C + q]);
  for (int q = 0; q < R_; ++q) blk->nmax_col = std::max(blk->nmax_col, mg.voff[q * C + c + 1] - mg.voff[q * C + c]);
  int64_t const ne = mg.ne, n_cols = C * blk->nmax_row, n_rows = R_ * blk->nmax_col;
  dbuf<int64_t> voff_d(P + 1, s);
  HIP_CHECK(hipMemcpyAsync(voff_d.data(), mg.voff.data(), (P + 1) * sizeof(int64_t), hipMemcpyHostToDevice, s));
  dbuf<uint32_t> rows(std::max<int64_t>(ne, 1), s), cols(std::max<int64_t>(ne, 1), s);
  if (ne)
    hipLaunchKernelGGL(k_mg_block_coo<V>, dim3(grid_for(ne, kBlock, 16384)), dim3(kBlock), 0, s, mg.src.data<V>(),
                       mg.dst.data<V>(), ne, voff_d.data(), P, C, blk->nmax_row, blk->nmax_col, rows.data(),
                       cols.data());
  CGX_LAUNCH_CHECK();
  int K = 1;
  if (R_ > 1) {
    K = h.tune.mg_chunks > 0 ? h.tune.mg_chunks : 1;
    K = (int)std::min<int64_t>(K, std::max<int64_t>(blk->nmax_col, 1));
  }
  blk->K  = K;
  blk->cs = std::max<int64_t>((blk->nmax_col + K - 1) / K, 1);
  blk->ch.resize(K);
  int64_t const n_rows_k = R_ * blk->cs;
  R const* const w_in    = g.weighted ? mg.w.data<R>() : nullptr;
  (void)n_rows;
  if (K == 1) {
    build_push_from_coo<uint32_t, R>(s, rows.data(), cols.data(), w_in, ne, n_rows_k, n_cols, blk->ch[0].pp, h.tune,
                                     false, 0, R_ == 1 && sizeof(R) == 4);
  } else {
    dbuf<uint32_t> chunk(ne, s), chunk_s(ne, s), iv(ne, s), perm(ne, s), rows_s(ne, s), cols_s(ne, s);
    dbuf<R> w_s(w_in ? ne : 1, s);
    hipLaunchKernelGGL(k_mg_row_chunks, dim3(grid_for(ne, kBlock, 16384)), dim3(kBlock), 0, s, rows.data(), ne,
                       blk->nmax_col, blk->cs, chunk.data());
    CGX_LAUNCH_CHECK();
    iota<uint32_t>(iv.data(), ne, 0u, s);
    radix_sort_pairs<uint32_t, uint32_t>(chunk.data(), chunk_s.data(), iv.data(), perm.data(), ne, 0,
                                         bits_for((unsigned long long)K), s);
    gather<uint32_t, uint32_t>(rows_s.data(), rows.data(), perm.data(), ne, s);
    gather<uint32_t, uint32_t>(cols_s.data(), cols.data(), perm.data(), ne, s);
    if (w_in) gather<R, uint32_t>(w_s.data(), w_in, perm.data(), ne, s);
    dbuf<int64_t> st_d(K + 1, s);
// ... 394 lines not shown
```

cugraph-forked_amd/pylibcugraph/__init__.py:

```python
from __future__ import annotations

import ctypes

from . import _lib
from ._arrays import (DeviceArray, DeviceView, copy_view_to_tensor, copy_views_to_tensors, optional_view,
                      to_device_tensor, views_to_tensors_owned, vptr)

from . import generators
from . import comms

__all__ = ["trim_device_cache", "ResourceHandle", "GraphProperties", "SGGraph", "MGGraph", "pagerank",
           "personalized_pagerank", "katz_centrality", "eigenvector_centrality", "hits", "bfs", "sssp",
           "louvain", "weakly_connected_components", "strongly_connected_components", "triangle_count",
           "version"]


def allocator_stats():
    out = (ctypes.c_double * 5)()
    _lib.lib.cugraph_amd_allocator_stats(out)
    return {"mallocs": int(out[0]), "malloc_bytes": int(out[1]), "malloc_s": out[2], "oom_trims": int(out[3]),
            "cached_bytes": int(out[4])}


def trim_device_cache():
    return int(_lib.lib.cugraph_amd_trim_device_cache())


def version():
    return _lib.lib.cugraph_amd_version().decode()


class ResourceHandle:

    def __init__(self, handle=None):
        p = None if handle is None else ctypes.c_void_p(int(handle))
        self.c_resource_handle_ptr = _lib.lib.cugraph_create_resource_handle(p)
        if not self.c_resource_handle_ptr:
            raise RuntimeError("cugraph_create_resource_handle failed")

    @property
    def ptr(self):
        return self.c_resource_handle_ptr

    def get_rank(self):
        return _lib.lib.cugraph_resource_handle_get_rank(self.c_resource_handle_ptr)

    def set_profiling(self, enable=True):
        _lib.lib.cugraph_amd_set_profiling(self.c_resource_handle_ptr, 1 if enable else 0)

    def set_option(self, name, value):
        if name is None:
            name, value = "defaults", 0
        _lib.call("cugraph_amd_set_option", self.c_resource_handle_ptr, name.encode(), float(value))

    def last_iterations(self):
        return _lib.lib.cugraph_amd_last_iterations(self.c_resource_handle_ptr)

    def last_hot_kernel_ms(self):
        return _lib.lib.cugraph_amd_last_hot_kernel_ms(self.c_resource_handle_ptr)

    def last_hot_kernel_launches(self):
        return _lib.lib.cugraph_amd_last_hot_kernel_launches(self.c_resource_handle_ptr)

    def last_bfs_levels(self):
        return _lib.lib.cugraph_amd_last_bfs_levels(self.c_resource_handle_ptr)

    def last_bfs_bottom_up_steps(self):
        return _lib.lib.cugraph_amd_last_bfs_bottom_up_steps(self.c_resource_handle_ptr)

    def last_louvain_levels(self):
        return _lib.lib.cugraph_amd_last_louvain_levels(self.c_resource_handle_ptr)

    def last_louvain_sweep_bytes(self):
        return _lib.lib.cugraph_amd_last_louvain_sweep_bytes(self.c_resource_handle_ptr)

    def last_louvain_partition(self):
        e, g = ctypes.c_int64(), ctypes.c_int64()
        _lib.lib.cugraph_amd_last_louvain_partition(self.c_resource_handle_ptr, ctypes.byref(e), ctypes.byref(g))
        return e.value, g.value

    def last_pagerank_schedule(self):
        n, m = ctypes.c_int64(), ctypes.c_int64()
        _lib.lib.cugraph_amd_last_pagerank_schedule(self.c_resource_handle_ptr, ctypes.byref(n), ctypes.byref(m))
        return n.value, m.value

    def measure_copy_bandwidth(self, nbytes=4 << 30, reps=10):
        r = _lib.lib.cugraph_amd_measure_copy_bandwidth(self.c_resource_handle_ptr, int(nbytes), int(reps))
        if r < 0:
            raise RuntimeError("cugraph_amd_measure_copy_bandwidth failed")
        return r

    def __del__(self, _sd=_lib.SHUTDOWN, _free=_lib.lib.cugraph_free_resource_handle):
        p = getattr(self, "c_resource_handle_ptr", None)
        if p and not _sd[0]:
            _free(p)
            self.c_resource_handle_ptr = None


class GraphProperties:

    def __init__(self, is_symmetric=False, is_multigraph=False):
        self.is_symmetric = bool(is_symmetric)
        self.is_multigraph = bool(is_multigraph)

    def _c(self):
        return _lib.GraphPropertiesStruct(int(self.is_symmetric), int(self.is_multigraph))

    def __getnewargs_ex__(self):
        return ((), {"is_symmetric": self.is_symmetric, "is_multigraph": self.is_multigraph})


class _GPUGraph:
    c_graph_ptr = None

    def number_of_vertices(self):
        return _lib.lib.cugraph_amd_graph_get_number_of_vertices(self.c_graph_ptr)

    def number_of_edges(self):
        return _lib.lib.cugraph_amd_graph_get_number_of_edges(self.c_graph_ptr)

    def adjacency(self, resource_handle, transposed=False):
        o, i, w = ctypes.c_void_p(), ctypes.c_void_p(), ctypes.c_void_p()
        _lib.call("cugraph_amd_graph_get_adjacency", resource_handle.ptr, self.c_graph_ptr,
                  1 if transposed else 0, ctypes.byref(o), ctypes.byref(i), ctypes.byref(w))
        h = resource_handle.ptr
        out = (DeviceArray(o.value).to_tensor(h), DeviceArray(i.value).to_tensor(h),
               DeviceArray(w.value).to_tensor(h) if w.value else None)
        return out

    def out_weight_sums(self, resource_handle):
        a = ctypes.c_void_p()
        _lib.call("cugraph_amd_graph_get_out_weight_sums", resource_handle.ptr, self.c_graph_ptr, ctypes.byref(a))
        return DeviceArray(a.value).to_tensor(resource_handle.ptr)


def _check_bool(name, v):
    if not isinstance(v, (int, bool)):
        raise TypeError(f"expected int or bool for {name}, got {type(v)}")


class SGGraph(_GPUGraph):

    def __init__(self, resource_handle, graph_properties, src_array, dst_array, weight_array,
                 store_transposed=False, renumber=False, do_expensive_check=False,
                 edge_id_array=None, edge_type_array=None):
        _check_bool("store_transposed", store_transposed)
        _check_bool("renumber", renumber)
        _check_bool("do_expensive_check", do_expensive_check)
        if edge_id_array is not None or edge_type_array is not None:
            raise NotImplementedError("edge ids / edge types are not supported by this build")
        src = DeviceView(src_array)
        dst = DeviceView(dst_array)
        if dst.c_type != src.c_type:
            dst = DeviceView(dst.tensor.to(src.tensor.dtype))
        wgt = optional_view(weight_array)
        props = graph_properties._c()
        g = ctypes.c_void_p()
        _lib.call("cugraph_sg_graph_create", resource_handle.ptr, ctypes.byref(props), src.ptr, dst.ptr,
                  vptr(wgt), None, None, int(bool(store_transposed)), int(bool(renumber)),
                  int(bool(do_expensive_check)), ctypes.byref(g))
        self.c_graph_ptr = g.value
        self._mg = False

    def __del__(self, _sd=_lib.SHUTDOWN, _free=_lib.lib.cugraph_sg_graph_free):
        if getattr(self, "c_graph_ptr", None) and not _sd[0]:
            _free(self.c_graph_ptr)
            self.c_graph_ptr = None


class MGGraph(_GPUGraph):

    def __init__(self, resource_handle, graph_properties, src_array, dst_array, weight_array,
                 store_transposed=False, num_edges=-1, do_expensive_check=False,
                 edge_id_array=None, edge_type_array=None):
        _check_bool("store_transposed", store_transposed)
        src = DeviceView(src_array)
        dst = DeviceView(dst_array, src.tensor.dtype)
        wgt = optional_view(weight_array)
        if num_edges < 0:
            raise ValueError("num_edges (global edge count) is required for MGGraph")
        props = graph_properties._c()
        g = ctypes.c_void_p()
        _lib.call("cugraph_mg_graph_create", resource_handle.ptr, ctypes.byref(props), src.ptr, dst.ptr,
                  vptr(wgt), None, None, int(bool(store_transposed)), int(num_edges),
                  int(bool(do_expensive_check)), ctypes.byref(g))
        self.c_graph_ptr = g.value
        self._mg = True

    def __del__(self, _sd=_lib.SHUTDOWN, _free=_lib.lib.cugraph_mg_graph_free):
        if getattr(self, "c_graph_ptr", None) and not _sd[0]:
            _free(self.c_graph_ptr)
            self.c_graph_ptr = None


def _centrality(api, resource_handle, graph, *views_and_scalars):
    res = ctypes.c_void_p()
    _lib.call(api, resource_handle.ptr, graph.c_graph_ptr, *views_and_scalars, ctypes.byref(res))
    v, x = views_to_tensors_owned(resource_handle.ptr, [_lib.lib.cugraph_centrality_result_get_vertices(res),
                                                        _lib.lib.cugraph_centrality_result_get_values(res)],
                                  res, _lib.lib.cugraph_centrality_result_free)
    return v, x


def pagerank(resource_handle, graph, precomputed_vertex_out_weight_vertices,
             precomputed_vertex_out_weight_sums, initial_guess_vertices, initial_guess_values,
             alpha, epsilon, max_iterations, do_expensive_check):
    a = optional_view(precomputed_vertex_out_weight_vertices)
    b = optional_view(precomputed_vertex_out_weight_sums)
    c = optional_view(initial_guess_vertices)
    d = optional_view(initial_guess_values)
    return _centrality("cugraph_pagerank", resource_handle, graph, vptr(a), vptr(b), vptr(c), vptr(d),
                       float(alpha), float(epsilon), int(max_iterations), int(bool(do_expensive_check)))


def personalized_pagerank(resource_handle, graph, precomputed_vertex_out_weight_vertices,
                          precomputed_vertex_out_weight_sums, initial_guess_vertices,
                          initial_guess_values, personalization_vertices, personalization_values,
                          alpha, epsilon, max_iterations, do_expensive_check):
    a = optional_view(precomputed_vertex_out_weight_vertices)
    b = optional_view(precomputed_vertex_out_weight_sums)
    c = optional_view(initial_guess_vertices)
    d = optional_view(initial_guess_values)
    e = optional_view(personalization_vertices)
    f = optional_view(personalization_values)
    return _centrality("cugraph_personalized_pagerank", resource_handle, graph, vptr(a), vptr(b), vptr(c),
                       vptr(d), vptr(e), vptr(f), float(alpha), float(epsilon), int(max_iterations),
                       int(bool(do_expensive_check)))


def _paths(resource_handle, res):
    v, d, p = views_to_tensors_owned(resource_handle.ptr, [_lib.lib.cugraph_paths_result_get_vertices(res),
                                                           _lib.lib.cugraph_paths_result_get_distances(res),
                                                           _lib.lib.cugraph_paths_result_get_predecessors(res)],
                                     res, _lib.lib.cugraph_paths_result_free)
    return v, d, p

# ... 170 lines not shown
```

cugraph-forked_amd/pylibcugraph/_lib.py:

```python
from __future__ import annotations

import atexit
import ctypes
import os

_HERE = os.path.dirname(os.path.abspath(__file__))
LIB_PATH = os.environ.get(
    "CUGRAPH_AMD_LIB", os.path.join(os.path.dirname(_HERE), "lib", "libcugraph_c.so"))

if not os.path.exists(LIB_PATH):
    raise ImportError(
        f"libcugraph_c.so not found at {LIB_PATH}: build it with "
        "`python -c 'import __graft_entry__ as g; g.build()'` (or `make -C cugraph-forked_amd`)")

try:
    import torch
except ImportError:
    torch = None

lib = ctypes.CDLL(LIB_PATH, mode=ctypes.RTLD_GLOBAL)

SHUTDOWN = [False]
atexit.register(lambda: SHUTDOWN.__setitem__(0, True))

INT32, INT64, FLOAT32, FLOAT64 = 0, 1, 2, 3
CODES = {
    0: "CUGRAPH_SUCCESS", 1: "CUGRAPH_UNKNOWN_ERROR", 2: "CUGRAPH_INVALID_HANDLE",
    3: "CUGRAPH_ALLOC_ERROR", 4: "CUGRAPH_INVALID_INPUT", 5: "CUGRAPH_NOT_IMPLEMENTED",
    6: "CUGRAPH_UNSUPPORTED_TYPE_COMBINATION",
}

P = ctypes.c_void_p
PP = ctypes.POINTER(ctypes.c_void_p)
c_size_t = ctypes.c_size_t
c_int = ctypes.c_int
c_double = ctypes.c_double


class GraphPropertiesStruct(ctypes.Structure):
    _fields_ = [("is_symmetric", ctypes.c_int), ("is_multigraph", ctypes.c_int)]


def _proto(name, restype, *argtypes):
    f = getattr(lib, name)
    f.restype = restype
    f.argtypes = list(argtypes)
    return f


_proto("cugraph_create_resource_handle", P, P)
_proto("cugraph_free_resource_handle", None, P)
_proto("cugraph_resource_handle_get_rank", c_int, P)
_proto("cugraph_error_message", ctypes.c_char_p, P)
_proto("cugraph_error_free", None, P)
_proto("cugraph_type_erased_device_array_create", c_int, P, c_size_t, c_int, PP, PP)
_proto("cugraph_type_erased_device_array_free", None, P)
_proto("cugraph_type_erased_device_array_view", P, P)
_proto("cugraph_type_erased_device_array_view_create", P, P, c_size_t, c_int)
_proto("cugraph_type_erased_device_array_view_free", None, P)
_proto("cugraph_type_erased_device_array_view_size", c_size_t, P)
_proto("cugraph_type_erased_device_array_view_type", c_int, P)
_proto("cugraph_type_erased_device_array_view_pointer", P, P)
_proto("cugraph_type_erased_device_array_view_copy", c_int, P, P, P, PP)
_proto("cugraph_type_erased_device_array_view_copy_to_host", c_int, P, P, P, PP)
_proto("cugraph_type_erased_device_array_view_copy_from_host", c_int, P, P, P, PP)
_proto("cugraph_sg_graph_create", c_int, P, ctypes.POINTER(GraphPropertiesStruct), P, P, P, P, P,
       c_int, c_int, c_int, PP, PP)
_proto("cugraph_sg_graph_free", None, P)
_proto("cugraph_mg_graph_create", c_int, P, ctypes.POINTER(GraphPropertiesStruct), P, P, P, P, P,
       c_int, c_size_t, c_int, PP, PP)
_proto("cugraph_mg_graph_free", None, P)
_proto("cugraph_pagerank", c_int, P, P, P, P, P, P, c_double, c_double, c_size_t, c_int, PP, PP)
_proto("cugraph_personalized_pagerank", c_int, P, P, P, P, P, P, P, P, c_double, c_double, c_size_t,
       c_int, PP, PP)
_proto("cugraph_centrality_result_get_vertices", P, P)
_proto("cugraph_centrality_result_get_values", P, P)
_proto("cugraph_centrality_result_free", None, P)
_proto("cugraph_katz_centrality", c_int, P, P, P, c_double, c_double, c_double, c_size_t, c_int, PP, PP)
_proto("cugraph_eigenvector_centrality", c_int, P, P, c_double, c_size_t, c_int, PP, PP)
_proto("cugraph_hits", c_int, P, P, c_double, c_size_t, P, P, c_int, c_int, PP, PP)
_proto("cugraph_hits_result_get_vertices", P, P)
_proto("cugraph_hits_result_get_hubs", P, P)
_proto("cugraph_hits_result_get_authorities", P, P)
_proto("cugraph_hits_result_get_hub_score_differences", c_double, P)
_proto("cugraph_hits_result_get_number_of_iterations", c_size_t, P)
_proto("cugraph_hits_result_free", None, P)
_proto("cugraph_extract_paths", c_int, P, P, P, P, P, PP, PP)
_proto("cugraph_extract_paths_result_get_max_path_length", c_size_t, P)
_proto("cugraph_extract_paths_result_get_paths", P, P)
_proto("cugraph_extract_paths_result_free", None, P)
_proto("cugraph_bfs", c_int, P, P, P, c_int, c_size_t, c_int, c_int, PP, PP)
_proto("cugraph_sssp", c_int, P, P, c_size_t, c_double, c_int, c_int, PP, PP)
_proto("cugraph_paths_result_get_vertices", P, P)
_proto("cugraph_paths_result_get_distances", P, P)
_proto("cugraph_paths_result_get_predecessors", P, P)
_proto("cugraph_paths_result_free", None, P)
_proto("cugraph_weakly_connected_components", c_int, P, P, c_int, PP, PP)
_proto("cugraph_strongly_connected_components", c_int, P, P, c_int, PP, PP)
_proto("cugraph_labeling_result_get_vertices", P, P)
_proto("cugraph_labeling_result_get_labels", P, P)
_proto("cugraph_labeling_result_free", None, P)
_proto("cugraph_triangle_count", c_int, P, P, P, c_int, PP, PP)
_proto("cugraph_triangle_count_result_get_vertices", P, P)
_proto("cugraph_triangle_count_result_get_counts", P, P)
_proto("cugraph_triangle_count_result_free", None, P)
_proto("cugraph_louvain", c_int, P, P, c_size_t, c_double, c_int, PP, PP)
_proto("cugraph_heirarchical_clustering_result_get_vertices", P, P)
_proto("cugraph_heirarchical_clustering_result_get_clusters", P, P)
_proto("cugraph_heirarchical_clustering_result_get_modularity", c_double, P)
_proto("cugraph_heirarchical_clustering_result_free", None, P)
_proto("cugraph_amd_heirarchical_clustering_result_get_num_levels", c_size_t, P)
_proto("cugraph_amd_heirarchical_clustering_result_get_level", P, P, c_size_t)
_proto("cugraph_amd_generate_rmat_edgelist", c_int, P, c_size_t, c_size_t, c_double, c_double, c_double,
       ctypes.c_uint64, c_int, c_int, c_size_t, c_int, PP, PP, PP)
_proto("cugraph_amd_generate_edge_weights", c_int, P, c_size_t, ctypes.c_uint64, c_size_t, c_int, PP, PP)
_proto("cugraph_amd_symmetrize_dedup", c_int, P, P, P, P, c_int, PP, PP, PP, PP)
_proto("cugraph_amd_graph_get_number_of_vertices", ctypes.c_int64, P)
_proto("cugraph_amd_graph_get_number_of_edges", ctypes.c_int64, P)
_proto("cugraph_amd_graph_is_symmetric", c_int, P)
_proto("cugraph_amd_graph_get_adjacency", c_int, P, P, c_int, PP, PP, PP, PP)
_proto("cugraph_amd_graph_get_out_weight_sums", c_int, P, P, PP, PP)
_proto("cugraph_amd_device_array_views_copy", c_int, P, c_size_t, P, P, PP)
_proto("cugraph_amd_set_profiling", None, P, c_int)
_proto("cugraph_amd_set_option", c_int, P, ctypes.c_char_p, c_double, PP)
_proto("cugraph_amd_last_iterations", c_size_t, P)
_proto("cugraph_amd_last_hot_kernel_ms", c_double, P)
_proto("cugraph_amd_last_hot_kernel_launches", c_size_t, P)
_proto("cugraph_amd_last_bfs_levels", c_size_t, P)
_proto("cugraph_amd_last_bfs_bottom_up_steps", c_size_t, P)
_proto("cugraph_amd_last_louvain_levels", c_size_t, P)
_proto("cugraph_amd_last_louvain_sweep_bytes", c_double, P)
_proto("cugraph_amd_last_louvain_partition", None, P, ctypes.POINTER(ctypes.c_int64), ctypes.POINTER(ctypes.c_int64))
_proto("cugraph_amd_last_pagerank_schedule", None, P, ctypes.POINTER(ctypes.c_int64), ctypes.POINTER(ctypes.c_int64))
_proto("cugraph_amd_trim_device_cache", c_size_t)
_proto("cugraph_amd_allocator_stats", None, ctypes.POINTER(c_double))
_proto("cugraph_amd_version", ctypes.c_char_p)
_proto("cugraph_amd_measure_copy_bandwidth", c_double, P, c_size_t, c_int)
_proto("cugraph_type_erased_device_array_release", P, P)
_proto("cugraph_amd_comm_unique_id_size", c_size_t)
_proto("cugraph_amd_comm_get_unique_id", c_int, P, PP)
_proto("cugraph_amd_mg_context_create_rccl", c_int, P, c_int, c_int, c_int, PP, PP)
_proto("cugraph_amd_mg_context_create_ops", c_int, P, P, P, c_int, PP, PP)
_proto("cugraph_amd_mg_context_free", None, P)


def assert_success(code, err, api_name):
    if code == 0:
        return
    msg = lib.cugraph_error_message(err) if err else b""
    msg = msg.decode() if isinstance(msg, bytes) else str(msg)
    if err:
        lib.cugraph_error_free(err)
    code_str = CODES.get(code, str(code))
    text = f"non-success value returned from {api_name}: {code_str} {msg}"
    if code in (2, 4):
        raise ValueError(text)
    if code == 3:
        raise MemoryError(text)
    if code == 5:
        raise NotImplementedError(text)
    if code == 6:
        raise TypeError(text)
    raise RuntimeError(text)


def call(api_name, *args):
    err = ctypes.c_void_p()
    code = getattr(lib, api_name)(*args, ctypes.byref(err))
    assert_success(code, err.value, api_name)
```

include/cugraph_amd/ext.h:

```cpp
#pragma once
#include <cugraph_c/algorithms.h>

#ifdef __cplusplus
extern "C" {
#endif

cugraph_error_code_t cugraph_amd_generate_rmat_edgelist(const cugraph_resource_handle_t* handle,
                                                        size_t scale,
                                                        size_t num_edges,
                                                        double a,
                                                        double b,
                                                        double c,
                                                        uint64_t seed,
                                                        bool_t clip_and_flip,
                                                        bool_t scramble_vertex_ids,
                                                        size_t first_edge,
                                                        data_type_id_t vertex_dtype,
                                                        cugraph_type_erased_device_array_t** src,
                                                        cugraph_type_erased_device_array_t** dst,
                                                        cugraph_error_t** error);

cugraph_error_code_t cugraph_amd_generate_edge_weights(const cugraph_resource_handle_t* handle,
                                                       size_t num_edges,
                                                       uint64_t seed,
                                                       size_t first_edge,
                                                       data_type_id_t weight_dtype,
                                                       cugraph_type_erased_device_array_t** weights,
                                                       cugraph_error_t** error);

cugraph_error_code_t cugraph_amd_symmetrize_dedup(const cugraph_resource_handle_t* handle,
                                                  const cugraph_type_erased_device_array_view_t* src,
                                                  const cugraph_type_erased_device_array_view_t* dst,
                                                  const cugraph_type_erased_device_array_view_t* weights,
                                                  bool_t symmetrize,
                                                  cugraph_type_erased_device_array_t** src_out,
                                                  cugraph_type_erased_device_array_t** dst_out,
                                                  cugraph_type_erased_device_array_t** weights_out,
                                                  cugraph_error_t** error);

int64_t cugraph_amd_graph_get_number_of_vertices(const cugraph_graph_t* graph);
int64_t cugraph_amd_graph_get_number_of_edges(const cugraph_graph_t* graph);
bool_t cugraph_amd_graph_is_symmetric(const cugraph_graph_t* graph);

cugraph_error_code_t cugraph_amd_graph_get_adjacency(const cugraph_resource_handle_t* handle,
                                                     cugraph_graph_t* graph,
                                                     bool_t transposed,
                                                     cugraph_type_erased_device_array_t** offsets,
                                                     cugraph_type_erased_device_array_t** indices,
                                                     cugraph_type_erased_device_array_t** weights,
                                                     cugraph_error_t** error);

cugraph_error_code_t cugraph_amd_graph_get_out_weight_sums(const cugraph_resource_handle_t* handle,
                                                           cugraph_graph_t* graph,
                                                           cugraph_type_erased_device_array_t** sums,
                                                           cugraph_error_t** error);

cugraph_error_code_t cugraph_amd_device_array_views_copy(const cugraph_resource_handle_t* handle,
                                                         size_t n,
                                                         cugraph_type_erased_device_array_view_t* const* dst,
                                                         const cugraph_type_erased_device_array_view_t* const* src,
                                                         cugraph_error_t** error);

void cugraph_amd_set_profiling(cugraph_resource_handle_t* handle, bool_t enable);
size_t cugraph_amd_last_iterations(const cugraph_resource_handle_t* handle);
cugraph_error_code_t cugraph_amd_set_option(cugraph_resource_handle_t* handle, const char* name, double value,
                                            cugraph_error_t** error);
double cugraph_amd_last_hot_kernel_ms(const cugraph_resource_handle_t* handle);
size_t cugraph_amd_last_hot_kernel_launches(const cugraph_resource_handle_t* handle);
void cugraph_amd_last_pagerank_schedule(const cugraph_resource_handle_t* handle, int64_t* stream_entries,
                                        int64_t* permuted_vertices);
size_t cugraph_amd_last_bfs_levels(const cugraph_resource_handle_t* handle);
size_t cugraph_amd_last_bfs_bottom_up_steps(const cugraph_resource_handle_t* handle);
size_t cugraph_amd_last_louvain_levels(const cugraph_resource_handle_t* handle);
double cugraph_amd_last_louvain_sweep_bytes(const cugraph_resource_handle_t* handle);
void cugraph_amd_last_louvain_partition(const cugraph_resource_handle_t* handle, int64_t* local_edges,
                                        int64_t* ghosts);
size_t cugraph_amd_heirarchical_clustering_result_get_num_levels(cugraph_heirarchical_clustering_result_t* result);
cugraph_type_erased_device_array_view_t* cugraph_amd_heirarchical_clustering_result_get_level(
  cugraph_heirarchical_clustering_result_t* result, size_t level);

size_t cugraph_amd_trim_device_cache(void);

void cugraph_amd_allocator_stats(double* out);

double cugraph_amd_measure_copy_bandwidth(const cugraph_resource_handle_t* handle, size_t bytes, int reps);

const char* cugraph_amd_version(void);

#ifdef __cplusplus
}
#endif
```

Baseline: 931.5 billion.

## Add run-row layout for PageRank push where 64-entry rows share one source

The push PageRank build now detects aligned 64-entry rows whose entries all come from one source vertex inside a window. It splits these out into a separate run region that stores one source id per row. The push kernel handles run units first with a deeper prefetch pipeline: it reads one x value per row instead of a per-entry gather, then falls back to the normal gather loop for the remaining units. This trades extra build kernels, a host-side unit list and a synchronize for fewer x gathers on high-degree vertices. It is on by default for 14-bit windows and for 12-bit windows with encoding enabled.

Result: faster. 985.5 billion (median of 6 runs) (+5.8%).

```diff
diff --git a/cugraph-forked_amd/csrc/capi.hpp b/cugraph-forked_amd/csrc/capi.hpp
--- a/cugraph-forked_amd/csrc/capi.hpp
+++ b/cugraph-forked_amd/csrc/capi.hpp
@@ -28,6 +28,8 @@
   int pr_perm          = -1;
   int64_t pr_perm_cut  = -1;
   int pr_perm_span     = -1;
+  int pr_runs          = -1;
+  int64_t pr_run_min   = -1;
   int pr_share_div     = 0;
   bool pr_fast_build   = true;
   int mg_chunks        = 0;
@@ -63,6 +65,8 @@
   size_t last_hot_launches   = 0;
   int64_t last_pr_stream     = 0;
   int64_t last_pr_permuted   = 0;
+  int64_t last_pr_run_rows    = 0;
+  int64_t last_pr_run_entries = 0;
   size_t last_bfs_levels    = 0;
   size_t last_bfs_bottom_up  = 0;
   size_t last_louvain_levels = 0;
@@ -170,6 +174,8 @@
   buffer pos;
   int64_t perm_cut = 0;
   int64_t stream_len = 0;
+  buffer run_src;
+  int64_t run_rows = 0, run_entries = 0;
   int last_iters = 0;
   double last_alpha = -1.0, last_eps = -1.0;
 };
diff --git a/cugraph-forked_amd/csrc/capi_core.cpp b/cugraph-forked_amd/csrc/capi_core.cpp
--- a/cugraph-forked_amd/csrc/capi_core.cpp
+++ b/cugraph-forked_amd/csrc/capi_core.cpp
@@ -510,6 +510,13 @@
       CGX_INPUT(value >= -1 && value <= 65536, "Invalid input argument: pr_perm_span must be in [-1, 65536]");
       i32(t.pr_perm_span);
     }
+    else if (n == "pr_runs") {
+      CGX_INPUT(value == -1 || value == 0 || value == 1, "Invalid input argument: pr_runs must be -1, 0 or 1");
+      i32(t.pr_runs);
+    } else if (n == "pr_run_min") {
+      CGX_INPUT(value == -1 || value >= 64, "Invalid input argument: pr_run_min must be -1 or at least 64");
+      t.pr_run_min = (int64_t)value;
+    }
     else if (n == "pr_fast_build") b(t.pr_fast_build);
     else if (n == "pr_share_div") i32(t.pr_share_div);
     else if (n == "mg_chunks") i32(t.mg_chunks);
@@ -563,6 +570,12 @@
   *stream_entries    = H(handle)->last_pr_stream;
   *permuted_vertices = H(handle)->last_pr_permuted;
 }
+extern "C" void cugraph_amd_last_pagerank_runs(const cugraph_resource_handle_t* handle, int64_t* run_rows,
+                                               int64_t* run_entries)
+{
+  *run_rows    = H(handle)->last_pr_run_rows;
+  *run_entries = H(handle)->last_pr_run_entries;
+}
 extern "C" size_t cugraph_amd_last_bfs_levels(const cugraph_resource_handle_t* handle)
 {
   return H(handle)->last_bfs_levels;
diff --git a/cugraph-forked_amd/csrc/pagerank.hip b/cugraph-forked_amd/csrc/pagerank.hip
--- a/cugraph-forked_amd/csrc/pagerank.hip
+++ b/cugraph-forked_amd/csrc/pagerank.hip
@@ -412,6 +412,16 @@
 }
 constexpr int64_t kPermCut = int64_t(1) << 20;
 
+constexpr int64_t kRunMin = 64;
+inline bool push_runs_on(int win_bits, tuning_t const& tu)
+{
+  if (win_bits == 13) return false;
+  if (win_bits == 12 && !tu.pr_enc) return false;
+  if (tu.pr_runs >= 0) return tu.pr_runs != 0;
+  return win_bits == 14;
+}
+inline int64_t push_run_min(tuning_t const& tu) { return std::max<int64_t>(tu.pr_run_min > 0 ? tu.pr_run_min : kRunMin, 64); }
+
 inline int push_blocks(int win_bits) { return win_bits >= 14 ? kPushBlocks / 2 : kPushBlocks; }
 
 constexpr int64_t kShareDiv = 4;
@@ -421,6 +431,7 @@
   int64_t base;
   int64_t win;
 };
+constexpr uint32_t kRunPad = 0xffffffffu;
 
 template <typename V, typename E, typename R>
 struct push_args {
@@ -429,6 +440,7 @@
   R const* ew;
   uint16_t const* ent16;
   uint32_t const* seg_base;
+  uint32_t const* run_src;
   push_unit const* units;
   int64_t nunits;
   unsigned long long* acc;
@@ -882,6 +894,7 @@
   constexpr uint32_t kLow   = (1u << WB) - 1;
   constexpr int kRows       = kSegEntries / 64;
   static_assert(kRows == kPerThread, "a wave segment is one unit row per thread");
+  constexpr bool kRuns = WB != 13 && (WB >= 14 || ENC) && !BANDS && sizeof(V) == 4 && std::is_same<R, float>::value;
   constexpr bool kAcc32 = WB == 15;
   using acc_t           = typename std::conditional<kAcc32, uint32_t, unsigned long long>::type;
   __shared__ acc_t acc[kWin];
@@ -987,31 +1000,93 @@
         }
       }
     };
-    int64_t const u1 = ua + 1 < ub ? ua + 1 : ua;
-    int nA      = seg_n(ua);
-    int nB      = seg_n(u1);
-    uint32_t bB = __builtin_amdgcn_readfirstlane(sa.seg_base[u1 * kSegsPerUnit + wave]);
-    u32x4_t wA  = nt_load(seg_ptr(ua));
-    u32x4_t wB  = nt_load(seg_ptr(u1));
-    xw_t xA[kRows];
-    if (nA > 0) gather(wA, __builtin_amdgcn_readfirstlane(sa.seg_base[ua * kSegsPerUnit + wave]), xA);
-    for (int64_t un = ua; un < ub; ++un) {
-      bool const actB = un + 1 < ub && nB > 0;
-      xw_t xB[kRows];
-      if (actB) gather(wB, bB, xB);
-      int64_t const u2  = un + 2 < ub ? un + 2 : un;
-      int const n2      = seg_n(u2);
-      uint32_t const b2 = sa.seg_base[u2 * kSegsPerUnit + wave];
-      u32x4_t const e2  = nt_load(seg_ptr(u2));
-      __builtin_amdgcn_sched_barrier(0);
-      if (nA > 0) sum(wA, xA);
-      wA = wB;
-#pragma unroll
-      for (int j = 0; j < kRows; ++j) xA[j] = xB[j];
-      nA = actB ? nB : 0;
-      wB = e2;
-      nB = n2;
-      bB = __builtin_amdgcn_readfirstlane(b2);
+    int64_t um = ua;
+    if constexpr (kRuns) {
+      while (um < ub && units[um].base < 0) ++um;
+      if (um > ua) {
+        constexpr int kDepth = WB < 14 ? 1 : 4;
+        constexpr int kAhead = kDepth / 2;
+        u32x4_t wq[kDepth];
+        uint32_t sq[kDepth];
+        xw_t xq[kDepth];
+        int nq[kDepth];
+        auto issue = [&](int64_t u, int k) {
+          int64_t const uc = u < um ? u : um - 1;
+          nq[k] = u < um ? seg_n(uc) : 0;
+          wq[k] = nt_load(seg_ptr(uc));
+          sq[k] = nt_load(sa.run_src + (~units[uc].base + wave * kRows + (lane & 7)));
+        };
+        auto issue_x = [&](int k) { xq[k] = x[sq[k] == kRunPad ? 0u : sq[k]]; };
+        auto word_of = [&](xw_t v, int j) {
+          static_assert(sizeof(xw_t) == 4, "run rows: fp32 x~ words");
+          return __builtin_bit_cast(xw_t, __builtin_amdgcn_readlane(__builtin_bit_cast(int, v), j));
+        };
+        auto run_sum = [&](u32x4_t const& w, uint32_t sv, xw_t xv) {
+          [[maybe_unused]] uint32_t lo[kRows], old[kRows];
+          [[maybe_unused]] uint32_t* const cw = kAcc32 ? sa.carry + ((win & kWinMask) << WB) : nullptr;
+#pragma unroll
+          for (int j = 0; j < kRows; ++j) {
+            if constexpr (kAcc32) lo[j] = old[j] = 0u;
+            if ((uint32_t)__builtin_amdgcn_readlane((int)sv, j) == kRunPad) continue;
+            unsigned long long fix;
+            if constexpr (ENC) fix = dec_fixed(word_of(xv, j));
+            else fix = fixed_of(word_of(xv, j));
+            uint32_t const slot = entry(w, j);
+            if constexpr (kAcc32) {
+              lo[j]  = (uint32_t)fix;
+              old[j] = atomicAdd(&acc[slot], lo[j]);
+              if (fix >> 32) atomicAdd(cw + slot, (uint32_t)(fix >> 32));
+            } else {
+              atomicAdd(&acc[slot], fix);
+            }
+          }
+          if constexpr (kAcc32) {
+#pragma unroll
+            for (int j = 0; j < kRows; ++j)
+              if (old[j] > ~lo[j]) atomicAdd(cw + entry(w, j), 1u);
+          }
+        };
+#pragma unroll
+        for (int k = 0; k < kDepth; ++k) issue(ua + k, k);
+#pragma unroll
+        for (int k = 0; k < kAhead; ++k) issue_x(k);
+        for (int64_t un = ua; un < um; un += kDepth) {
+#pragma unroll
+          for (int k = 0; k < kDepth; ++k) {
+            issue_x((k + kAhead) % kDepth);
+            if (nq[k] > 0) run_sum(wq[k], sq[k], xq[k]);
+            issue(un + k + kDepth, k);
+          }
+        }
+      }
+    }
+    if (!kRuns || um < ub) {
+      int64_t const u1 = um + 1 < ub ? um + 1 : um;
+      int nA      = seg_n(um);
+      int nB      = seg_n(u1);
+      uint32_t bB = __builtin_amdgcn_readfirstlane(sa.seg_base[u1 * kSegsPerUnit + wave]);
+      u32x4_t wA  = nt_load(seg_ptr(um));
+      u32x4_t wB  = nt_load(seg_ptr(u1));
+      xw_t xA[kRows];
+      if (nA > 0) gather(wA, __builtin_amdgcn_readfirstlane(sa.seg_base[um * kSegsPerUnit + wave]), xA);
+      for (int64_t un = um; un < ub; ++un) {
+        bool const actB = un + 1 < ub && nB > 0;
+        xw_t xB[kRows];
+        if (actB) gather(wB, bB, xB);
+        int64_t const u2  = un + 2 < ub ? un + 2 : un;
+        int const n2      = seg_n(u2);
+        uint32_t const b2 = sa.seg_base[u2 * kSegsPerUnit + wave];
+        u32x4_t const e2  = nt_load(seg_ptr(u2));
+        __builtin_amdgcn_sched_barrier(0);
+        if (nA > 0) sum(wA, xA);
+        wA = wB;
+#pragma unroll
+        for (int j = 0; j < kRows; ++j) xA[j] = xB[j];
+        nA = actB ? nB : 0;
+        wB = e2;
+        nB = n2;
+        bB = __builtin_amdgcn_readfirstlane(b2);
+      }
     }
     end_item<WB, V, E, R, FUSE, BANDS>(sa, acc, win);
     if (sa.item_ticks && tid == 0) sa.item_ticks[s_item] = (uint32_t)(__builtin_amdgcn_s_memrealtime() - s_t0);
@@ -1021,8 +1096,7 @@
       if ((int64_t)k < sa.tl_cap) {
         unsigned long long* r = sa.tl + 1 + 4 * k;
         r[0] = ((unsigned long long)sa.launch << 32) | blockIdx.x;
-        int64_t const iu = s_item;
-        r[1] = ((unsigned long long)(units[sa.items[iu + 1] - 1].k1 - units[sa.items[iu]].k0) << 32) | (unsigned long long)iu;
+        r[1] = (unsigned long long)s_item;
         r[2] = s_t0;
         r[3] = t_end;
       }
@@ -1475,7 +1549,7 @@
     push_unit const u = units[i / kSegsPerUnit];
     int64_t const p   = u.k0 + (i % kSegsPerUnit) * kSegEntries;
     uint32_t base     = 0;
-    if (p < u.k1) {
+    if (p < u.k1 && u.base >= 0) {
       int64_t lo = 0, hi = ne - 1;
       while (lo < hi) {
         int64_t mid = (lo + hi) >> 1;
@@ -1495,6 +1569,118 @@
   }
 }
 
+constexpr int kFlagThreads = 1024, kFlagPer = 4, kFlagTile = kFlagThreads * kFlagPer;
+__global__ __launch_bounds__(kFlagThreads) void k_run_flags(uint64_t const* keys, int64_t ne, int wb, int64_t tmin,
+                                                            uint8_t* stays, uint32_t* tile_packed)
+{
+  __shared__ int64_t s_first0;
+  __shared__ int s_wave[kFlagThreads / 64];
+  __shared__ uint32_t s_packed;
+  int const t = threadIdx.x, lane = t & 63, wv = t >> 6;
+  for (int64_t k0 = blockIdx.x * (int64_t)kFlagTile; k0 < ne; k0 += (int64_t)gridDim.x * kFlagTile) {
+    if (t == 0) s_packed = 0;
+    if (wv == 0) {
+      uint64_t const g0 = keys[k0] >> wb;
+      int64_t hi        = k0;
+      auto back = [&](int64_t stride) {
+        int64_t const i = hi - stride * (lane + 1);
+        bool const same = i >= 0 && (keys[i] >> wb) == g0;
+        unsigned long long const m = __ballot(same);
+        int const j = m == ~0ull ? 64 : __builtin_ctzll(~m);
+        hi -= stride * j;
+        return j;
+      };
+      if (back(1) == 64) {
+        while (back(512) == 64) {}
+        back(8);
+        back(1);
+      }
+      if (lane == 0) s_first0 = hi;
+    }
+    int64_t const kt = k0 + (int64_t)kFlagPer * t;
+    uint64_t g[kFlagPer];
+    int hl = -1;
+    uint64_t prev = kt > 0 && kt <= ne ? keys[kt - 1] >> wb : 0;
+#pragma unroll
+    for (int i = 0; i < kFlagPer; ++i) {
+      g[i] = kt + i < ne ? keys[kt + i] >> wb : 0;
+      if (kt + i < ne && (kt + i == 0 || g[i] != prev)) hl = kFlagPer * t + i;
+      prev = g[i];
+    }
+    int h = hl;
+    for (int d = 1; d < 64; d <<= 1) {
+      int const o = __shfl_up(h, d);
+      if (lane >= d) h = max(h, o);
+    }
+    if (lane == 63) s_wave[wv] = h;
+    __syncthreads();
+    int he = __shfl_up(h, 1);
+    if (lane == 0) he = -1;
+    for (int i = 0; i < wv; ++i) he = max(he, s_wave[i]);
+    prev = kt > 0 && kt <= ne ? keys[kt - 1] >> wb : 0;
+#pragma unroll
+    for (int i = 0; i < kFlagPer; ++i) {
+      int64_t const k = kt + i;
+      if (k >= ne) break;
+      if (k == 0 || g[i] != prev) he = kFlagPer * t + i;
+      prev = g[i];
+      int64_t const first = he >= 0 ? k0 + he : s_first0;
+      int64_t const last  = k - ((k - first) & 63) + 63;
+      bool const row = last < ne && (keys[last] >> wb) == g[i] && first + tmin - 1 < ne && (keys[first + tmin - 1] >> wb) == g[i];
+      stays[k] = row ? 0 : 1;
+      if (!row) atomicAdd(&s_packed, 1u);
+    }
+    __syncthreads();
+    if (t == 0) tile_packed[k0 / kFlagTile] = s_packed;
+  }
+}
+
+__global__ __launch_bounds__(kFlagThreads) void k_run_split(uint64_t const* keys, int64_t ne, uint8_t const* stays,
+                                                            uint32_t const* tile_off, int64_t npk, uint64_t* out)
+{
+  __shared__ int s_wave[kFlagThreads / 64];
+  int const t = threadIdx.x, lane = t & 63, wv = t >> 6;
+  for (int64_t k0 = blockIdx.x * (int64_t)kFlagTile; k0 < ne; k0 += (int64_t)gridDim.x * kFlagTile) {
+    int64_t const kt = k0 + (int64_t)kFlagPer * t;
+    int f[kFlagPer], c = 0;
+#pragma unroll
+    for (int i = 0; i < kFlagPer; ++i) {
+      f[i] = kt + i < ne ? stays[kt + i] : 0;
+      c += f[i];
+    }
+    int h = c;
+    for (int d = 1; d < 64; d <<= 1) {
+      int const o = __shfl_up(h, d);
+      if (lane >= d) h += o;
+    }
+    if (lane == 63) s_wave[wv] = h;
+    __syncthreads();
+    int before = h - c;
+    for (int i = 0; i < wv; ++i) before += s_wave[i];
+    int64_t const off = (int64_t)tile_off[k0 / kFlagTile];
+    int64_t pp = off + before;
+    int64_t pr = npk + (k0 - off) + (kFlagPer * t - before);
+#pragma unroll
+    for (int i = 0; i < kFlagPer; ++i) {
+      if (kt + i >= ne) break;
+      out[f[i] ? pp++ : pr++] = keys[kt + i];
+    }
+    __syncthreads();
+  }
+}
+
+__global__ void k_run_pack(uint64_t const* rk, int64_t nrk, int64_t const* rws, int64_t const* rnws, key_p kc,
+                           uint16_t* ent_run, uint32_t* run_src)
+{
+  for (int64_t i = blockIdx.x * (int64_t)blockDim.x + threadIdx.x; i < nrk; i += (int64_t)gridDim.x * blockDim.x) {
+    uint64_t const key = rk[i];
+    int64_t const w    = kc.win(key);
+    int64_t const p    = rnws[w] + (i - rws[w]);
+    ent_run[seg_store_index(p)] = (uint16_t)kc.slot(key);
+    if ((p & 63) == 0) run_src[p >> 6] = kc.src(key);
+  }
+}
+
 inline void mark_whole_items(hipStream_t s, pr_push_t& pp, push_unit* units, std::vector<push_unit>& hu,
                              std::vector<int64_t> const& item_u, int64_t nitems, tuning_t const& tu)
 {
@@ -1561,20 +1747,21 @@
 inline void build_items(hipStream_t s, pr_push_t& pp, push_unit* units, int64_t nunits, bool xcd_queues,
                         tuning_t const& tu)
 {
-  int64_t const ne = nunits ? to_host(&units[nunits - 1].k1, 1, s)[0] : 0;
-  auto hu = to_host(units, nunits, s);
+  auto hu    = to_host(units, nunits, s);
+  int64_t ne = 0;
+  for (auto const& u : hu) ne += u.k1 - u.k0;
   int64_t const div = tu.pr_share_div > 0 ? tu.pr_share_div : kShareDiv;
   int64_t const tg  = std::max<int64_t>(kPushUnit, ne / (push_blocks(pp.win_bits) * div));
   std::vector<int64_t> item_u, item_e;
   for (int64_t u0 = 0; u0 < nunits;) {
     int64_t u1 = u0;
     while (u1 < nunits && hu[u1].win == hu[u0].win) ++u1;
-    int64_t const size = hu[u1 - 1].k1 - hu[u0].k0;
-    int64_t const n    = std::max<int64_t>(1, (size + tg / 2) / tg);
-    int64_t k          = 0;
-    for (int64_t u = u0; u < u1; ++u) {
-      int64_t const done = hu[u].k0 - hu[u0].k0;
-      bool const head    = u == u0 || (xcd_queues ? (k < n && done * n >= k * size) : (u - u0) % kTileUnits == 0);
+    int64_t size = 0;
+    for (int64_t u = u0; u < u1; ++u) size += hu[u].k1 - hu[u].k0;
+    int64_t const n = std::max<int64_t>(1, (size + tg / 2) / tg);
+    int64_t k = 0, done = 0;
+    for (int64_t u = u0; u < u1; done += hu[u].k1 - hu[u].k0, ++u) {
+      bool const head = u == u0 || (xcd_queues ? (k < n && done * n >= k * size) : (u - u0) % kTileUnits == 0);
       if (head) {
         item_u.push_back(u);
         item_e.push_back(0);
@@ -1933,7 +2120,7 @@
 
 template <typename E, typename CM>
 bool build_push_packed_sym_cm(hipStream_t s, E const* off, uint32_t const* idx, int64_t ne, int64_t nv, pr_push_t& pp,
-                              tuning_t const& tu, int64_t band_cut, bool wide)
+                              tuning_t const& tu, int64_t band_cut, bool wide, bool runs_ok)
 {
   int const wb = push_win_bits(nv, tu, wide);
   if (wb != 14 || band_cut >= nv) band_cut = 0;
@@ -1975,6 +2162,31 @@
       if (db.current() != kbuf.data()) std::swap(kbuf, k2);
     }
   }
+  int64_t const ne_all     = ne;
+  uint64_t const* rk_first = nullptr;
+  int64_t nrk              = 0;
+  if (band_cut == 0 && ne && runs_ok && push_runs_on(wb, tu)) {
+    int64_t const ntiles = (ne + kFlagTile - 1) / kFlagTile;
+    unsigned const grid  = (unsigned)std::min<int64_t>(ntiles, 1 << 16);
+    dbuf<uint8_t> stays(ne, s);
+    dbuf<uint32_t> tcnt(ntiles + 1, s), toff(ntiles + 1, s);
+    HIP_CHECK(hipMemsetAsync(tcnt.data() + ntiles, 0, sizeof(uint32_t), s));
+    hipLaunchKernelGGL(k_run_flags, dim3(grid), dim3(kFlagThreads), 0, s, kbuf.data(), ne, wb, push_run_min(tu),
+                       stays.data(), tcnt.data());
+    CGX_LAUNCH_CHECK();
+    exclusive_scan<uint32_t, uint32_t>(tcnt.data(), toff.data(), ntiles + 1, s);
+    int64_t const npk = (int64_t)to_host(toff.data() + ntiles, 1, s)[0];
+    nrk               = ne - npk;
+    if (nrk) {
+      dbuf<uint64_t> pk(ne, s);
+      hipLaunchKernelGGL(k_run_split, dim3(grid), dim3(kFlagThreads), 0, s, kbuf.data(), ne, stays.data(), toff.data(),
+                         npk, pk.data());
+      CGX_LAUNCH_CHECK();
+      std::swap(kbuf, pk);
+      rk_first = kbuf.data() + npk;
+      ne       = npk;
+    }
+  }
   uint64_t const* keys = kbuf.data();
   dbuf<int64_t> ws(nwin + 1, s);
   hipLaunchKernelGGL(k_win_starts<key_p>, dim3(grid_for(nwin + 1, kBlock, 4096)), dim3(kBlock), 0, s, keys, ne, nwin,
@@ -1997,7 +2209,7 @@
   CGX_LAUNCH_CHECK();
   exclusive_scan<unsigned long long, unsigned long long>(pad.data(), pb.data(), nwin + 1, s);
   int64_t const total = total0 + (int64_t)to_host(pb.data() + nwin, 1, s)[0];
-  if (!(total <= ne + ne / 2 && (uint64_t)total < (1ull << 32))) {
+  if (!(total + nrk <= ne_all + ne_all / 2 && (uint64_t)total < (1ull << 32))) {
     pp.pos.release();
     pp.perm_cut = 0;
     return false;
@@ -2026,9 +2238,41 @@
   pp.nitems = 0;
   pp.packed = true;
   uint16_t const pad_code = (uint16_t)(((1u << (16 - wb)) - 1) << wb);
+  std::vector<int64_t> h_rws, h_rnws;
+  int64_t run_off = 0, run_total = 0;
+  pp.run_rows = pp.run_entries = 0;
+  pp.run_src.release();
+  dbuf<int64_t> rws;
+  if (nrk) {
+    rws.resize(nwin + 1, s);
+    hipLaunchKernelGGL(k_win_starts<key_p>, dim3(grid_for(nwin + 1, kBlock, 4096)), dim3(kBlock), 0, s, rk_first,
+                       nrk, nwin, rws.data(), kc);
+    CGX_LAUNCH_CHECK();
+    h_rws = to_host(rws.data(), (size_t)(nwin + 1), s);
+    h_rnws.assign((size_t)(nwin + 1), 0);
+    for (int64_t w = 0; w < nwin; ++w)
+      h_rnws[w + 1] = h_rnws[w] + (h_rws[w + 1] - h_rws[w] + kSegEntries - 1) / kSegEntries * kSegEntries;
+    run_total       = h_rnws[nwin];
+    run_off         = (total + kPushUnit - 1) / kPushUnit * kPushUnit;
+    pp.run_rows     = nrk / 64;
+    pp.run_entries  = nrk;
+  }
+  int64_t const ent_len = (nrk ? run_off + run_total : total) + kPushUnit;
   pp.ent16.set_stream(s);
-  pp.ent16.resize((total + kPushUnit) * sizeof(uint16_t));
-  fill<uint16_t>(pp.ent16.data<uint16_t>(), (size_t)(total + kPushUnit), pad_code, s);
+  pp.ent16.resize(ent_len * sizeof(uint16_t));
+  fill<uint16_t>(pp.ent16.data<uint16_t>(), (size_t)ent_len, pad_code, s);
+  if (nrk) {
+    int64_t const nrows = run_total / 64 + kPushUnit / 64;
+    pp.run_src.set_stream(s);
+    pp.run_src.resize(nrows * sizeof(uint32_t));
+    fill<uint32_t>(pp.run_src.data<uint32_t>(), (size_t)nrows, kRunPad, s);
+    dbuf<int64_t> rnws(nwin + 1, s);
+    to_device(rnws.data(), h_rnws.data(), h_rnws.size(), s);
+    hipLaunchKernelGGL(k_run_pack, dim3(grid_for(nrk, kBlock, 16384)), dim3(kBlock), 0, s, rk_first, nrk, rws.data(),
+                       rnws.data(), kc, pp.ent16.data<uint16_t>() + run_off, pp.run_src.data<uint32_t>());
+    CGX_LAUNCH_CHECK();
+    HIP_CHECK(hipStreamSynchronize(s));
+  }
   if (ne)
     hipLaunchKernelGGL(k_pack16_p<CM>, dim3(grid_for(ne, kBlock, 16384)), dim3(kBlock), 0, s, keys, ne, ws.data(),
                        cm, pb.data(), kc, pmax, pp.ent16.data<uint16_t>());
@@ -2037,21 +2281,39 @@
   hipLaunchKernelGGL(k_packed_win_starts<CM>, dim3(grid_for(nwin + 1, kBlock, 4096)), dim3(kBlock), 0, s, ws.data(),
                      cm, pb.data(), nwin, total0, nws.data());
   CGX_LAUNCH_CHECK();
-  dbuf<uint32_t> ucnt(nwin + 1, s), upos(nwin + 1, s);
-  hipLaunchKernelGGL(k_unit_counts, dim3(grid_for(nwin + 1, kBlock, 4096)), dim3(kBlock), 0, s, nws.data(), nwin,
-                     ucnt.data());
-  CGX_LAUNCH_CHECK();
-  exclusive_scan<uint32_t, uint32_t>(ucnt.data(), upos.data(), nwin + 1, s);
-  int64_t const nunits = (int64_t)to_host(upos.data() + nwin, 1, s)[0];
+  int64_t nunits   = 0;
+  push_unit* units = nullptr;
   pp.units.set_stream(s);
-  pp.units.resize(std::max<int64_t>(nunits, 1) * sizeof(push_unit));
-  push_unit* units = pp.units.data<push_unit>();
-  if (nunits)
-    hipLaunchKernelGGL(k_units_direct, dim3(grid_for(nunits, kBlock, 4096)), dim3(kBlock), 0, s, nws.data(), nwin,
-                       upos.data(), nunits, units);
-  CGX_LAUNCH_CHECK();
-  hipLaunchKernelGGL(k_unit_ends, dim3(grid_for(nunits, kBlock, 4096)), dim3(kBlock), 0, s, units, nunits, total);
-  CGX_LAUNCH_CHECK();
+  if (nrk) {
+    auto const h_nws = to_host(nws.data(), (size_t)(nwin + 1), s);
+    std::vector<push_unit> hu;
+    for (int64_t w = 0; w < nwin; ++w) {
+      for (int64_t p = h_rnws[w]; p < h_rnws[w + 1]; p += kPushUnit)
+        hu.push_back(push_unit{run_off + p, run_off + std::min<int64_t>(p + kPushUnit, h_rnws[w + 1]), ~(p / 64), w});
+      for (int64_t p = h_nws[w]; p < h_nws[w + 1]; p += kPushUnit)
+        hu.push_back(push_unit{p, std::min<int64_t>(p + kPushUnit, h_nws[w + 1]), 0, w});
+    }
+    nunits = (int64_t)hu.size();
+    pp.units.resize(std::max<int64_t>(nunits, 1) * sizeof(push_unit));
+    units = pp.units.data<push_unit>();
+    to_device(units, hu.data(), hu.size(), s);
+    HIP_CHECK(hipStreamSynchronize(s));
+  } else {
+    dbuf<uint32_t> ucnt(nwin + 1, s), upos(nwin + 1, s);
+    hipLaunchKernelGGL(k_unit_counts, dim3(grid_for(nwin + 1, kBlock, 4096)), dim3(kBlock), 0, s, nws.data(), nwin,
+                       ucnt.data());
+    CGX_LAUNCH_CHECK();
+    exclusive_scan<uint32_t, uint32_t>(ucnt.data(), upos.data(), nwin + 1, s);
+    nunits = (int64_t)to_host(upos.data() + nwin, 1, s)[0];
+    pp.units.resize(std::max<int64_t>(nunits, 1) * sizeof(push_unit));
+    units = pp.units.data<push_unit>();
+    if (nunits)
+      hipLaunchKernelGGL(k_units_direct, dim3(grid_for(nunits, kBlock, 4096)), dim3(kBlock), 0, s, nws.data(), nwin,
+                         upos.data(), nunits, units);
+    CGX_LAUNCH_CHECK();
+    hipLaunchKernelGGL(k_unit_ends, dim3(grid_for(nunits, kBlock, 4096)), dim3(kBlock), 0, s, units, nunits, total);
+    CGX_LAUNCH_CHECK();
+  }
   pp.seg_base.set_stream(s);
   pp.seg_base.resize(std::max<int64_t>(nunits * kSegsPerUnit, 1) * sizeof(uint32_t));
   if (nunits)
@@ -2069,10 +2331,11 @@
 
 template <typename E>
 bool build_push_packed_sym(hipStream_t s, E const* off, uint32_t const* idx, int64_t ne, int64_t nv, pr_push_t& pp,
-                           tuning_t const& tu, int64_t band_cut, bool wide)
-{
-  if (ne < (int64_t(1) << 31)) return build_push_packed_sym_cm<E, uint32_t>(s, off, idx, ne, nv, pp, tu, band_cut, wide);
-  return build_push_packed_sym_cm<E, unsigned long long>(s, off, idx, ne, nv, pp, tu, band_cut, wide);
+                           tuning_t const& tu, int64_t band_cut, bool wide, bool runs_ok)
+{
+  if (ne < (int64_t(1) << 31))
+    return build_push_packed_sym_cm<E, uint32_t>(s, off, idx, ne, nv, pp, tu, band_cut, wide, runs_ok);
+  return build_push_packed_sym_cm<E, unsigned long long>(s, off, idx, ne, nv, pp, tu, band_cut, wide, runs_ok);
 }
 
 template <typename V, typename E, typename R>
@@ -2089,7 +2352,8 @@
   if constexpr (sizeof(V) == 4) {
     if (g.symmetric && !use_weights && h.tune.pr_packed && h.tune.pr_fast_build &&
         build_push_packed_sym<E>(s, adj.offsets.data<E>(), reinterpret_cast<uint32_t const*>(adj.indices.data<V>()), ne,
-                                 nv, adj.pr, h.tune, push_band_cut(nv, h.tune), sizeof(R) == 4))
+                                 nv, adj.pr, h.tune, push_band_cut(nv, h.tune), sizeof(R) == 4,
+                                 sizeof(R) == 4))
       return;
   }
   dbuf<uint32_t> rows(std::max<int64_t>(ne, 1), s);
@@ -2151,6 +2415,7 @@
   sa.ew       = pp.ew.empty() ? nullptr : pp.ew.data<R>();
   sa.ent16    = pp.ent16.data<uint16_t>();
   sa.seg_base = pp.seg_base.data<uint32_t>();
+  sa.run_src  = pp.run_src.empty() ? nullptr : pp.run_src.data<uint32_t>();
   sa.units    = pp.units.data<push_unit>();
   sa.nunits   = pp.nunits;
   sa.acc      = pp.acc.data<unsigned long long>();
@@ -2321,11 +2586,14 @@
   a.x_in     = nullptr;
   a.x_out    = xa.data();
 
-  a.enc  = push && adj.pr.packed && std::is_same<R, float>::value && h.tune.pr_enc;
+  a.enc  = push && adj.pr.packed && std::is_same<R, float>::value &&
+          (h.tune.pr_enc || (adj.pr.win_bits == 12 && adj.pr.run_rows > 0));
   a.fp64 = push ? 0 : 1;
   a.pos  = push && adj.pr.perm_cut ? adj.pr.pos.data<uint32_t>() : nullptr;
   h.last_pr_stream   = push ? adj.pr.stream_len : 0;
   h.last_pr_permuted = push && adj.pr.perm_cut ? nv - adj.pr.perm_cut : 0;
+  h.last_pr_run_rows    = push ? adj.pr.run_rows : 0;
+  h.last_pr_run_entries = push ? adj.pr.run_entries : 0;
   hipLaunchKernelGGL((k_pr_init<V, E, R>), dim3(nblk_init), dim3(kBlock), 0, s, a);
   CGX_LAUNCH_CHECK();
 
@@ -2424,8 +2692,10 @@
       auto hi = to_host(adj.pr.items.data<int64_t>(), adj.pr.nitems + 1, s);
       for (unsigned long long i = 0; i < n; ++i) {
         unsigned long long const it = rec[4 * i + 1] & 0xffffffffull;
-        std::fprintf(f, "%llu,%llu,%llu,%llu,%lld,%llu,%llu\n", rec[4 * i] >> 32, rec[4 * i] & 0xffffffffull, it,
-                     rec[4 * i + 1] >> 32, (long long)(hu[hi[it]].win & kWinMask), rec[4 * i + 2], rec[4 * i + 3]);
+        long long ents = 0;
+        for (int64_t u = hi[it]; u < hi[it + 1]; ++u) ents += hu[u].k1 - hu[u].k0;
+        std::fprintf(f, "%llu,%llu,%llu,%lld,%lld,%llu,%llu\n", rec[4 * i] >> 32, rec[4 * i] & 0xffffffffull, it, ents,
+                     (long long)(hu[hi[it]].win & kWinMask), rec[4 * i + 2], rec[4 * i + 3]);
       }
       std::fclose(f);
     }
diff --git a/cugraph-forked_amd/pylibcugraph/__init__.py b/cugraph-forked_amd/pylibcugraph/__init__.py
--- a/cugraph-forked_amd/pylibcugraph/__init__.py
+++ b/cugraph-forked_amd/pylibcugraph/__init__.py
@@ -82,6 +82,11 @@
     def last_pagerank_schedule(self):
         n, m = ctypes.c_int64(), ctypes.c_int64()
         _lib.lib.cugraph_amd_last_pagerank_schedule(self.c_resource_handle_ptr, ctypes.byref(n), ctypes.byref(m))
+        return n.value, m.value
+
+    def last_pagerank_runs(self):
+        n, m = ctypes.c_int64(), ctypes.c_int64()
+        _lib.lib.cugraph_amd_last_pagerank_runs(self.c_resource_handle_ptr, ctypes.byref(n), ctypes.byref(m))
         return n.value, m.value
 
     def measure_copy_bandwidth(self, nbytes=4 << 30, reps=10):
diff --git a/cugraph-forked_amd/pylibcugraph/_lib.py b/cugraph-forked_amd/pylibcugraph/_lib.py
--- a/cugraph-forked_amd/pylibcugraph/_lib.py
+++ b/cugraph-forked_amd/pylibcugraph/_lib.py
@@ -132,6 +132,7 @@
 _proto("cugraph_amd_last_louvain_sweep_bytes", c_double, P)
 _proto("cugraph_amd_last_louvain_partition", None, P, ctypes.POINTER(ctypes.c_int64), ctypes.POINTER(ctypes.c_int64))
 _proto("cugraph_amd_last_pagerank_schedule", None, P, ctypes.POINTER(ctypes.c_int64), ctypes.POINTER(ctypes.c_int64))
+_proto("cugraph_amd_last_pagerank_runs", None, P, ctypes.POINTER(ctypes.c_int64), ctypes.POINTER(ctypes.c_int64))
 _proto("cugraph_amd_trim_device_cache", c_size_t)
 _proto("cugraph_amd_allocator_stats", None, ctypes.POINTER(c_double))
 _proto("cugraph_amd_version", ctypes.c_char_p)
diff --git a/include/cugraph_amd/ext.h b/include/cugraph_amd/ext.h
--- a/include/cugraph_amd/ext.h
+++ b/include/cugraph_amd/ext.h
@@ -69,6 +69,7 @@
 size_t cugraph_amd_last_hot_kernel_launches(const cugraph_resource_handle_t* handle);
 void cugraph_amd_last_pagerank_schedule(const cugraph_resource_handle_t* handle, int64_t* stream_entries,
                                         int64_t* permuted_vertices);
+void cugraph_amd_last_pagerank_runs(const cugraph_resource_handle_t* handle, int64_t* run_rows, int64_t* run_entries);
 size_t cugraph_amd_last_bfs_levels(const cugraph_resource_handle_t* handle);
 size_t cugraph_amd_last_bfs_bottom_up_steps(const cugraph_resource_handle_t* handle);
 size_t cugraph_amd_last_louvain_levels(const cugraph_resource_handle_t* handle);
```
